# ndlongvn/MM-DTI

Measured on AMD Instinct MI355X. Metric: molecules/sec fwd+bwd (InfoNCE fine-tune), higher is better.
Workload: dtype fp16 forward / bf16 backward GEMM operands, fp32 accumulation

## Files before the change

### mm-dti_amd/csrc/gbf.hip

```cpp
#include "common.h"

namespace mmdti {

constexpr float GBF_A = 2.5066272160f;

__global__ __launch_bounds__(256) void gbf_fwd_kernel(const float* __restrict__ dist, const long long* __restrict__ et,
                                                      const float* __restrict__ mul, const float* __restrict__ bias,
                                                      const float* __restrict__ means, const float* __restrict__ stds,
                                                      long long P, int K, int E, bf16_t* __restrict__ feat) {
  const int kc = threadIdx.x & 15;
  const int pl = threadIdx.x >> 4;
  for (int k0 = kc * 8; k0 < K; k0 += 128) {
    float mu[8], sg[8], cf[8];
#pragma unroll
    for (int i = 0; i < 8; ++i) {
      mu[i] = means[k0 + i];
      sg[i] = fabsf(stds[k0 + i]) + 1e-5f;
      cf[i] = 1.0f / (GBF_A * sg[i]);
    }
    for (long long p = (long long)blockIdx.x * 16 + pl; p < P; p += (long long)gridDim.x * 16) {
      long long e = et[p];
      e = e < 0 ? 0 : (e >= E ? E - 1 : e);
      const float y = mul[e] * dist[p] + bias[e];
      uint32_t w[4];
#pragma unroll
      for (int i = 0; i < 4; ++i) {
        float z0 = (y - mu[2 * i]) / sg[2 * i], z1 = (y - mu[2 * i + 1]) / sg[2 * i + 1];
        float v0 = __expf(-0.5f * z0 * z0) * cf[2 * i], v1 = __expf(-0.5f * z1 * z1) * cf[2 * i + 1];
        w[i] = (uint32_t)f2bf(v0) | ((uint32_t)f2bf(v1) << 16);
      }
      *reinterpret_cast<uint4*>(feat + p * K + k0) = make_uint4(w[0], w[1], w[2], w[3]);
    }
  }
}

constexpr int GBF_MAXE = 4096;

__global__ __launch_bounds__(256) void gbf_bwd_kernel(const float* __restrict__ dist, const long long* __restrict__ et,
                                                      const float* __restrict__ mul, const float* __restrict__ bias,
                                                      const float* __restrict__ means, const float* __restrict__ stds,
                                                      long long P, int K, int E, const bf16_t* __restrict__ dfeat,
                                                      float* __restrict__ dmul, float* __restrict__ dbias,
                                                      float* __restrict__ dmeans, float* __restrict__ dstds) {
  extern __shared__ float hist[];
  const bool use_hist = E <= GBF_MAXE;
  if (use_hist) {
    for (int i = threadIdx.x; i < 2 * E; i += 256) hist[i] = 0.f;
    __syncthreads();
  }
  const int kc = threadIdx.x & 15, pl = threadIdx.x >> 4;
  for (int kb = 0; kb < K; kb += 128) {
    const int k0 = kb + kc * 8;
    const bool kact = k0 < K;
    float mu[8], sg[8], cf[8], amu[8], asg[8];
#pragma unroll
    for (int i = 0; i < 8; ++i) {
      mu[i] = kact ? means[k0 + i] : 0.f;
      sg[i] = kact ? fabsf(stds[k0 + i]) + 1e-5f : 1.f;
      cf[i] = 1.0f / (GBF_A * sg[i]);
      amu[i] = asg[i] = 0.f;
    }
    for (long long p0 = (long long)blockIdx.x * 16; p0 < P; p0 += (long long)gridDim.x * 16) {
      const long long p = p0 + pl;
      float dy = 0.f;
      long long e = 0;
      float d = 0.f;
      if (p < P && kact) {
        e = et[p];
        e = e < 0 ? 0 : (e >= E ? E - 1 : e);
        d = dist[p];
        const float y = mul[e] * d + bias[e];
        const uint4 u = *reinterpret_cast<const uint4*>(dfeat + p * K + k0);
        const uint32_t w[4] = {u.x, u.y, u.z, u.w};
#pragma unroll
        for (int i = 0; i < 8; ++i) {
          const float dv = __uint_as_float((i & 1) ? (w[i >> 1] & 0xffff0000u) : (w[i >> 1] << 16));
          const float z = (y - mu[i]) / sg[i];
          const float val = __expf(-0.5f * z * z) * cf[i];
          const float t = dv * val;
          const float zs = z / sg[i];
          dy -= t * zs;
          amu[i] += t * zs;
          asg[i] += t * (z * zs - 1.0f / sg[i]);
        }
      }
      dy += __shfl_xor(dy, 1, 64);
      dy += __shfl_xor(dy, 2, 64);
      dy += __shfl_xor(dy, 4, 64);
      dy += __shfl_xor(dy, 8, 64);
      if (kc == 0 && p < P) {
        if (use_hist) {
          atomicAdd(&hist[e], dy * d);
          atomicAdd(&hist[E + e], dy);
        } else {
          atomicAdd(dmul + e, dy * d);
          atomicAdd(dbias + e, dy);
        }
      }
    }
#pragma unroll
    for (int i = 0; i < 8; ++i) {
      float a = amu[i], s = asg[i];
      a += __shfl_xor(a, 16, 64); a += __shfl_xor(a, 32, 64);
      s += __shfl_xor(s, 16, 64); s += __shfl_xor(s, 32, 64);
      if ((threadIdx.x & 63) < 16 && kact) {
        atomicAdd(dmeans + k0 + i, a);
        atomicAdd(dstds + k0 + i, stds[k0 + i] < 0.f ? -s : s);
      }
    }
  }
  if (use_hist) {
    __syncthreads();
    for (int i = threadIdx.x; i < E; i += 256) {
      const float a = hist[i], b = hist[E + i];
      if (a != 0.f) atomicAdd(dmul + i, a);
      if (b != 0.f) atomicAdd(dbias + i, b);
    }
  }
}

__global__ __launch_bounds__(256) void pair_permute_fwd_kernel(const float* __restrict__ x, float* __restrict__ out,
                                                               int N, int H, int ld) {
  extern __shared__ float tile[];
  const int bi = blockIdx.x, b = bi / N, i = bi - b * N;
  const float* src = x + (long long)bi * N * H;
  const int HP = H + 1;
  for (int t = threadIdx.x; t < N * H; t += 256) tile[(t / H) * HP + (t % H)] = src[t];
  __syncthreads();
  for (int t = threadIdx.x; t < H * N; t += 256) {
    const int h = t / N, j = t - h * N;
    out[(((long long)b * H + h) * N + i) * ld + j] = tile[j * HP + h];
  }
}

__global__ __launch_bounds__(256) void pair_permute_bwd_kernel(const float* __restrict__ g, bf16_t* __restrict__ out,
                                                               int N, int H, int ld, int tiled) {
  extern __shared__ float tile[];
  const int bi = blockIdx.x, b = bi / N, i = bi - b * N;
  const int NP = N | 1;
  for (int t = threadIdx.x; t < H * N; t += 256) {
    const int h = t / N, j = t - h * N;
    const long long off = tiled ? (long long)(b * H + h) * pair_plane(N) + pair_off(N, i, j) : (((long long)b * H + h) * N + i) * ld + j;
    tile[h * NP + j] = g[off];
  }
  __syncthreads();
  bf16_t* dst = out + (long long)bi * N * H;
  for (int t = threadIdx.x; t < N * H; t += 256) {
    const int j = t / H, h = t - j * H;
    dst[t] = f2bf(tile[h * NP + j]);
  }
}

typedef __bf16 gbf16x8 __attribute__((ext_vector_type(8)));
typedef float gf32x4 __attribute__((ext_vector_type(4)));
constexpr int GBF_K = 128, GBF_F = 128, GBF_H = 64;
constexpr int GBF_WS = 136;

__device__ __forceinline__ gbf16x8 gbf_pack8(const float* v) {
  gbf16x8 r;
#pragma unroll
  for (int e = 0; e < 8; ++e) r[e] = (__bf16)v[e];
  return r;
}
__device__ __forceinline__ uint2 gbf_pack4(const gf32x4& a) {
  uint2 pk;
  pk.x = (uint32_t)f2bf(a[0]) | ((uint32_t)f2bf(a[1]) << 16);
  pk.y = (uint32_t)f2bf(a[2]) | ((uint32_t)f2bf(a[3]) << 16);
  return pk;
}

__device__ __forceinline__ int gbf_edge(const void* et, long long base, unsigned off, int esz) {
  const char* pb = reinterpret_cast<const char*>(et) + base * esz;
  const unsigned bo = off * (unsigned)esz;
  const int w = *reinterpret_cast<const int*>(pb + (bo & ~3u));
  return esz == 2 ? (int)(short)(w >> ((bo & 2u) * 8u)) : w;
}
__device__ __forceinline__ int gbf_edge(const void* et, long long p, int esz) { return gbf_edge(et, p, 0u, esz); }

typedef float gf32x2 __attribute__((ext_vector_type(2)));
constexpr float GBF_SQ = 0.84932180028801907f;

__device__ __forceinline__ gbf16x8 gbf_basis8(float y, const float* mu, const float* isq, const float* cf) {
  const gf32x4 m0 = *reinterpret_cast<const gf32x4*>(mu), m1 = *reinterpret_cast<const gf32x4*>(mu + 4);
  const gf32x4 s0 = *reinterpret_cast<const gf32x4*>(isq), s1 = *reinterpret_cast<const gf32x4*>(isq + 4);
  const gf32x4 c0 = *reinterpret_cast<const gf32x4*>(cf), c1 = *reinterpret_cast<const gf32x4*>(cf + 4);
  const gf32x2 yy = {y, y};
  float v[8];
#define GBF_B2(M, S, C, LO, OUT)                                                       \
  {                                                                                    \
    const gf32x2 z = (yy - gf32x2{M[LO], M[LO + 1]}) * gf32x2{S[LO], S[LO + 1]};       \
    const gf32x2 q = -(z * z);                                                         \
    const gf32x2 e = {__builtin_amdgcn_exp2f(q[0]), __builtin_amdgcn_exp2f(q[1])};     \
    const gf32x2 r = e * gf32x2{C[LO], C[LO + 1]};                                     \
    v[OUT] = r[0]; v[OUT + 1] = r[1];                                                  \
  }
  GBF_B2(m0, s0, c0, 0, 0) GBF_B2(m0, s0, c0, 2, 2) GBF_B2(m1, s1, c1, 0, 4) GBF_B2(m1, s1, c1, 2, 6)
#undef GBF_B2
  return gbf_pack8(v);
}

constexpr int GBF_FWD_MAXE = 4096;
__device__ __forceinline__ void gbf_put(float* p, float v) { *p = v; }
__device__ __forceinline__ void gbf_put(_Float16* p, float v) { *p = (_Float16)fminf(v, 65504.f); }
__device__ __forceinline__ float gbf_get(const float* p) { return *p; }
__device__ __forceinline__ float gbf_get(const __bf16* p) {
  return __builtin_bit_cast(float, (uint32_t)(*reinterpret_cast<const unsigned short*>(p)) << 16);
}

template <bool SAVE, bool TILED, typename OT>
__global__ __launch_bounds__(512, 2) void gbf_bias_fwd_kernel(const float* __restrict__ dist, const void* __restrict__ et, int esz,
                                                              const float* __restrict__ mul, const float* __restrict__ bias,
                                                              const float* __restrict__ means, const float* __restrict__ stds,
                                                              const bf16_t* __restrict__ W1, const float* __restrict__ b1,
                                                              const bf16_t* __restrict__ W2, const float* __restrict__ b2,
                                                              OT* __restrict__ out, bf16_t* __restrict__ feat_out,
                                                              bf16_t* __restrict__ u_out, bf16_t* __restrict__ h_out, int B, int N,
                                                              int ld, int E, int tpm, int ugrad, int ltab,
                                                              const int* __restrict__ tile_prefix, const int* __restrict__ row_blocks) {
  static_assert(TILED || sizeof(OT) == 4, "compact pair planes exist in the tiled layout only");
  extern __shared__ __attribute__((aligned(16))) unsigned char gbf_smem[];
  bf16_t* sW1 = reinterpret_cast<bf16_t*>(gbf_smem);
  bf16_t* sW2 = sW1 + GBF_F * GBF_WS;
  float* sMu = reinterpret_cast<float*>(sW2 + GBF_H * GBF_WS);
  float* sIq = sMu + GBF_K;
  float* sCf = sIq + GBF_K;
  float* sB1 = sCf + GBF_K;
  float* sB2 = sB1 + GBF_F;
  float* sMul = sB2 + GBF_H;
  float* sBia = sMul + E;
  const int tid = threadIdx.x, lane = tid & 63;
  for (int c = tid; c < GBF_F * (GBF_K / 8); c += 512) {
    const int row = c >> 4, col = (c & 15) * 8;
    *reinterpret_cast<uint4*>(sW1 + row * GBF_WS + col) = *reinterpret_cast<const uint4*>(W1 + row * GBF_K + col);
  }
  for (int c = tid; c < GBF_H * 32; c += 512) {
    const int row = c >> 5, pc = c & 31, u = pc >> 3, g = (pc >> 1) & 3, hf = pc & 1;
    *reinterpret_cast<uint2*>(sW2 + row * GBF_WS + 32 * u + 8 * g + 4 * hf) =
        *reinterpret_cast<const uint2*>(W2 + row * GBF_F + 32 * u + 16 * hf + 4 * g);
  }
  if (tid < GBF_K) {
    const float sg = fabsf(stds[tid]) + 1e-5f;
    sMu[tid] = means[tid];
    sIq[tid] = GBF_SQ / sg;
    sCf[tid] = 1.0f / (GBF_A * sg);
    sB1[tid] = b1[tid];
    if (tid < GBF_H) sB2[tid] = b2[tid];
  }
  if (ltab)
    for (int c = tid; c < E; c += 512) {
      sMul[c] = mul[c];
      sBia[c] = bias[c];
    }
  __syncthreads();
  const int g = lane >> 4, i = lane & 15;
  const bool rag = TILED && tile_prefix != nullptr;
  const int ntiles = rag ? tile_prefix[B] : B * tpm;
  const int nwaves = (int)gridDim.x * 8;
  int b_run = 0;
  const int nblk = (N + 3) >> 2;
  const long long plane = TILED ? pair_plane(N) : (long long)N * ld;
  auto fetch = [&](int tile, int& b, int& q, int& flags, unsigned& pl, int& e, float& d) {
    tile = __builtin_amdgcn_readfirstlane(tile < ntiles ? tile : ntiles - 1);
    int tq;
    if (rag) {
      while (b_run + 1 < B && tile >= tile_prefix[b_run + 1]) ++b_run;
      b = b_run;
      tq = tile - tile_prefix[b];
    } else {
      b = (int)((unsigned)tile / (unsigned)tpm);
      tq = tile - b * tpm;
    }
    int ii, jj;
    bool inplane = true, past = false;
    if (TILED) {
      const int rbk = (rag && row_blocks) ? row_blocks[b] : nblk;
      const int cb = (int)((unsigned)tq / (unsigned)rbk), rb = tq - cb * rbk;
      past = 4 * rb >= N || 4 * cb >= N;
      ii = 4 * rb + (i >> 2);
      jj = 4 * cb + (i & 3);
      inplane = ii < N;
      q = (int)pair_off(N, inplane ? ii : 0, jj);
    } else {
      q = tq * 16 + i;
      ii = (int)((unsigned)q / (unsigned)ld);
      jj = q - ii * ld;
      inplane = q < plane;
    }
    const bool valid = ii < N && jj < N;
    flags = (valid ? 1 : 0) | (inplane ? 2 : 0) | (past ? 4 : 0);
    pl = (unsigned)((valid ? ii : 0) * N + (valid ? jj : 0));
    const long long mol = (long long)b * N * N;
    const int e32 = gbf_edge(et, mol, pl, esz);
    e = e32 < 0 ? 0 : (e32 >= E ? E - 1 : e32);
    d = (dist + mol)[pl];
  };
  int b, q, flags, e, n_b, n_q, n_flags, n_e;
  unsigned pl, n_pl;
  float d, n_d;
  int tile = (int)blockIdx.x * 8 + (tid >> 6);
  fetch(tile, b, q, flags, pl, e, d);
  for (; tile < ntiles; tile += nwaves) {
    fetch(tile + nwaves, n_b, n_q, n_flags, n_pl, n_e, n_d);
    const bool valid = flags & 1, inplane = flags & 2, past = flags & 4;
    const float padv = TILED ? -INFINITY : 0.f;
    OT* ob = out + (long long)b * GBF_H * plane + q;
    if (TILED && past) {
    } else {
    const long long p = (long long)b * N * N + pl;
    const float y = ltab ? sMul[e] * d + sBia[e] : mul[e] * d + bias[e];
    gbf16x8 fB[4];
#pragma unroll
    for (int c = 0; c < 4; ++c) {
      const int k0 = 32 * c + 8 * g;
      fB[c] = gbf_basis8(y, sMu + k0, sIq + k0, sCf + k0);
      if (SAVE && valid) *reinterpret_cast<gbf16x8*>(feat_out + p * GBF_K + k0) = fB[c];
    }
    gbf16x8 hB[4];
#pragma unroll
    for (int u = 0; u < 4; ++u) {
      gf32x4 hv[2];
#pragma unroll
      for (int hf = 0; hf < 2; ++hf) {
        const int ft = 2 * u + hf;
        gf32x4 acc = {0.f, 0.f, 0.f, 0.f};
#pragma unroll
        for (int c = 0; c < 4; ++c) {
          const gbf16x8 wf = *reinterpret_cast<const gbf16x8*>(sW1 + (16 * ft + i) * GBF_WS + 32 * c + 8 * g);
          acc = __builtin_amdgcn_mfma_f32_16x16x32_bf16(wf, fB[c], acc, 0, 0, 0);
        }
        const gf32x4 bb = *reinterpret_cast<const gf32x4*>(sB1 + 16 * ft + 4 * g);
        acc += bb;
        if (SAVE && ugrad) {
          f32x2_t y0, g0, y1, g1;
          gelu_erf_both2(f32x2_t{acc[0], acc[1]}, y0, g0);
          gelu_erf_both2(f32x2_t{acc[2], acc[3]}, y1, g1);
          acc = gf32x4{y0[0], y0[1], y1[0], y1[1]};
          const gf32x4 gq = {g0[0], g0[1], g1[0], g1[1]};
          if (valid) *reinterpret_cast<uint2*>(u_out + p * GBF_F + 16 * ft + 4 * g) = gbf_pack4(gq);
        } else {
          if (SAVE && valid) *reinterpret_cast<uint2*>(u_out + p * GBF_F + 16 * ft + 4 * g) = gbf_pack4(acc);
          const f32x2_t y0 = gelu_erf2(f32x2_t{acc[0], acc[1]}), y1 = gelu_erf2(f32x2_t{acc[2], acc[3]});
          acc = gf32x4{y0[0], y0[1], y1[0], y1[1]};
        }
        if (SAVE && valid) *reinterpret_cast<uint2*>(h_out + p * GBF_F + 16 * ft + 4 * g) = gbf_pack4(acc);
        hv[hf] = acc;
        __builtin_amdgcn_sched_barrier(0);
      }
      float v[8] = {hv[0][0], hv[0][1], hv[0][2], hv[0][3], hv[1][0], hv[1][1], hv[1][2], hv[1][3]};
      hB[u] = gbf_pack8(v);
    }
#pragma unroll
    for (int ht = 0; ht < 4; ++ht) {
      gf32x4 acc = {0.f, 0.f, 0.f, 0.f};
#pragma unroll
      for (int u = 0; u < 4; ++u) {
        const gbf16x8 wf = *reinterpret_cast<const gbf16x8*>(sW2 + (16 * ht + i) * GBF_WS + 32 * u + 8 * g);
        acc = __builtin_amdgcn_mfma_f32_16x16x32_bf16(wf, hB[u], acc, 0, 0, 0);
      }
      const gf32x4 bb = *reinterpret_cast<const gf32x4*>(sB2 + 16 * ht + 4 * g);
      if (inplane) {
#pragma unroll
        for (int r = 0; r < 4; ++r) gbf_put(ob + (long long)(16 * ht + 4 * g + r) * plane, valid ? acc[r] + bb[r] : padv);
      }
      __builtin_amdgcn_sched_barrier(0);
    }
    }
    b = n_b; q = n_q; flags = n_flags; pl = n_pl; e = n_e; d = n_d;
  }
}

constexpr int GBF_W2S = 72;

template <bool TILED, typename GT>
__global__ __launch_bounds__(256, 2) void gbf_bias_bwd_kernel(const GT* __restrict__ gsrc, const float* __restrict__ dist,
                                                           const void* __restrict__ et, int esz, const float* __restrict__ mul,
                                                           const float* __restrict__ bias, const float* __restrict__ means,
                                                           const float* __restrict__ stds, const bf16_t* __restrict__ W1,
                                                           const bf16_t* __restrict__ W2, const bf16_t* __restrict__ u_in,
                                                           bf16_t* __restrict__ do_out, bf16_t* __restrict__ du_out,
                                                           float* __restrict__ dmul, float* __restrict__ dbias,
                                                           float* __restrict__ dmeans, float* __restrict__ dstds, int B, int N, int ld,
                                                           int E, int tpm, int ugrad) {
  extern __shared__ __attribute__((aligned(16))) unsigned char gbf_smem[];
  bf16_t* sW1T = reinterpret_cast<bf16_t*>(gbf_smem);
  bf16_t* sW2T = sW1T + GBF_K * GBF_WS;
  float* sMu = reinterpret_cast<float*>(sW2T + GBF_F * GBF_W2S);
  float* sIs = sMu + GBF_K;
  float* sCf = sIs + GBF_K;
  float* hist = sCf + GBF_K;
  float* sMul = hist + 2 * E;
  float* sBia = sMul + E;
  const int tid = threadIdx.x, lane = tid & 63;
  for (int c = tid; c < E; c += 256) {
    sMul[c] = mul[c];
    sBia[c] = bias[c];
  }
  for (int c = tid; c < GBF_K * GBF_F; c += 256) {
    const int f = c >> 7, k = c & 127;
    const int u = f >> 5, hf = (f >> 4) & 1, g = (f >> 2) & 3, e = f & 3;
    sW1T[k * GBF_WS + 32 * u + 8 * g + 4 * hf + e] = W1[c];
  }
  for (int c = tid; c < GBF_H * GBF_F; c += 256) {
    const int h = c >> 7, f = c & 127;
    sW2T[f * GBF_W2S + h] = W2[c];
  }
  if (tid < GBF_K) {
    const float sg = fabsf(stds[tid]) + 1e-5f;
    sMu[tid] = means[tid];
    sIs[tid] = 1.0f / sg;
    sCf[tid] = 1.0f / (GBF_A * sg);
  }
  for (int c = tid; c < 2 * E; c += 256) hist[c] = 0.f;
  __syncthreads();
  const int g = lane >> 4, i = lane & 15;
  const long long ntiles = (long long)B * tpm;
  const long long nwaves = (long long)gridDim.x * 4;
  const int nblk = (N + 3) >> 2;
  const long long plane = TILED ? pair_plane(N) : (long long)N * ld;
  gf32x4 amu[8], asg[8];
#pragma unroll
  for (int kt = 0; kt < 8; ++kt) amu[kt] = asg[kt] = gf32x4{0.f, 0.f, 0.f, 0.f};
  auto fetch = [&](long long tile, bool& act, bool& valid, long long& p, int& e, float& d, float (&gv)[16], uint2 (&up)[8]) {
    act = false;
    valid = false;
    p = 0;
    e = 0;
    d = 0.f;
    if (tile >= ntiles) return;
    const int b = (int)(tile / tpm);
    const int tq = (int)(tile - (long long)b * tpm);
    int q, ii, jj;
    if (TILED) {
      const int rb = tq / nblk, cb = tq - rb * nblk;
      if (4 * rb >= N || 4 * cb >= N) return;
      ii = 4 * rb + (i >> 2);
      jj = 4 * cb + (i & 3);
      q = (int)pair_off(N, ii < N ? ii : 0, jj);
    } else {
      q = tq * 16 + i;
      ii = q / ld;
      jj = q - ii * ld;
    }
    act = true;
    valid = ii < N && jj < N;
    p = ((long long)b * N + (valid ? ii : 0)) * N + (valid ? jj : 0);
    const int e32 = gbf_edge(et, p, esz);
    e = e32 < 0 ? 0 : (e32 >= E ? E - 1 : e32);
    d = dist[p];
    const GT* gp = gsrc + (long long)b * GBF_H * plane + (valid ? q : 0);
#pragma unroll
    for (int c = 0; c < 2; ++c)
#pragma unroll
      for (int j = 0; j < 8; ++j) gv[c * 8 + j] = valid ? gbf_get(gp + (long long)(32 * c + 8 * g + j) * plane) : 0.f;
#pragma unroll
    for (int ft = 0; ft < 8; ++ft) {
      up[ft] = make_uint2(0u, 0u);
      if (valid) up[ft] = *reinterpret_cast<const uint2*>(u_in + p * GBF_F + 16 * ft + 4 * g);
    }
  };
  bool act, valid, n_act, n_valid;
  long long p, n_p;
  int e, n_e;
  float d, n_d, gv[16], n_gv[16];
  uint2 upre[8], n_up[8];
  long long tile = (long long)blockIdx.x * 4 + (tid >> 6);
  fetch(tile, act, valid, p, e, d, gv, upre);
  for (; tile < ntiles; tile += nwaves) {
    fetch(tile + nwaves, n_act, n_valid, n_p, n_e, n_d, n_gv, n_up);
    if (act) {
    const float y = sMul[e] * d + sBia[e];
    gbf16x8 oB[2];
#pragma unroll
    for (int c = 0; c < 2; ++c) {
      oB[c] = gbf_pack8(gv + 8 * c);
      if (valid) *reinterpret_cast<gbf16x8*>(do_out + p * GBF_H + 32 * c + 8 * g) = oB[c];
    }
    gbf16x8 uB[4];
#pragma unroll
    for (int u = 0; u < 4; ++u) {
      gf32x4 dv[2];
#pragma unroll
      for (int hf = 0; hf < 2; ++hf) {
        const int ft = 2 * u + hf;
        gf32x4 acc = {0.f, 0.f, 0.f, 0.f};
#pragma unroll
        for (int c = 0; c < 2; ++c) {
          const gbf16x8 wf = *reinterpret_cast<const gbf16x8*>(sW2T + (16 * ft + i) * GBF_W2S + 32 * c + 8 * g);
          acc = __builtin_amdgcn_mfma_f32_16x16x32_bf16(wf, oB[c], acc, 0, 0, 0);
        }
        const uint2 up = upre[ft];
        if (ugrad) {
          acc[0] *= __uint_as_float(up.x << 16);
          acc[1] *= __uint_as_float(up.x & 0xffff0000u);
          acc[2] *= __uint_as_float(up.y << 16);
          acc[3] *= __uint_as_float(up.y & 0xffff0000u);
        } else {
          acc[0] *= gelu_erf_grad(__uint_as_float(up.x << 16));
          acc[1] *= gelu_erf_grad(__uint_as_float(up.x & 0xffff0000u));
          acc[2] *= gelu_erf_grad(__uint_as_float(up.y << 16));
          acc[3] *= gelu_erf_grad(__uint_as_float(up.y & 0xffff0000u));
        }
        if (valid) *reinterpret_cast<uint2*>(du_out + p * GBF_F + 16 * ft + 4 * g) = gbf_pack4(acc);
        dv[hf] = acc;
        __builtin_amdgcn_sched_barrier(0);
      }
      float v[8] = {dv[0][0], dv[0][1], dv[0][2], dv[0][3], dv[1][0], dv[1][1], dv[1][2], dv[1][3]};
      uB[u] = gbf_pack8(v);
    }
    float dy = 0.f;
#pragma unroll
    for (int kt = 0; kt < 8; ++kt) {
      gf32x4 acc = {0.f, 0.f, 0.f, 0.f};
#pragma unroll
      for (int u = 0; u < 4; ++u) {
        const gbf16x8 wf = *reinterpret_cast<const gbf16x8*>(sW1T + (16 * kt + i) * GBF_WS + 32 * u + 8 * g);
        acc = __builtin_amdgcn_mfma_f32_16x16x32_bf16(wf, uB[u], acc, 0, 0, 0);
      }
      const gf32x4 mu = *reinterpret_cast<const gf32x4*>(sMu + 16 * kt + 4 * g);
      const gf32x4 is = *reinterpret_cast<const gf32x4*>(sIs + 16 * kt + 4 * g);
      const gf32x4 cf = *reinterpret_cast<const gf32x4*>(sCf + 16 * kt + 4 * g);
#pragma unroll
      for (int r = 0; r < 4; ++r) {
        const float dvr = __uint_as_float(((uint32_t)f2bf(acc[r])) << 16);
        const float z = (y - mu[r]) * is[r];
        const float val = __expf(-0.5f * z * z) * cf[r];
        const float t = valid ? dvr * val : 0.f;
        const float zs = z * is[r];
        dy -= t * zs;
        amu[kt][r] += t * zs;
        asg[kt][r] += t * (z * zs - is[r]);
      }
      __builtin_amdgcn_sched_barrier(0);
    }
    dy += __shfl_xor(dy, 16, 64);
    dy += __shfl_xor(dy, 32, 64);
    if (g == 0 && valid) {
      atomicAdd(&hist[e], dy * d);
      atomicAdd(&hist[E + e], dy);
    }
    }
    act = n_act; valid = n_valid; p = n_p; e = n_e; d = n_d;
#pragma unroll
    for (int j = 0; j < 16; ++j) gv[j] = n_gv[j];
#pragma unroll
    for (int j = 0; j < 8; ++j) upre[j] = n_up[j];
  }
#pragma unroll
  for (int kt = 0; kt < 8; ++kt)
#pragma unroll
    for (int r = 0; r < 4; ++r) {
      float a = amu[kt][r], sgv = asg[kt][r];
      a += __shfl_xor(a, 1, 64); a += __shfl_xor(a, 2, 64); a += __shfl_xor(a, 4, 64); a += __shfl_xor(a, 8, 64);
      sgv += __shfl_xor(sgv, 1, 64); sgv += __shfl_xor(sgv, 2, 64); sgv += __shfl_xor(sgv, 4, 64); sgv += __shfl_xor(sgv, 8, 64);
      if (i == 0) {
        const int k = 16 * kt + 4 * g + r;
        atomicAdd(dmeans + k, a);
        atomicAdd(dstds + k, stds[k] < 0.f ? -sgv : sgv);
      }
    }
  __syncthreads();
  for (int c = tid; c < E; c += 256) {
    const float a = hist[c], bb = hist[E + c];
    if (a != 0.f) atomicAdd(dmul + c, a);
    if (bb != 0.f) atomicAdd(dbias + c, bb);
  }
}

constexpr int GBF_LW = 144;
constexpr int GBF_FULL_MAXE = 1536;
constexpr int GBF_SLAB_B1 = GBF_F * GBF_K + GBF_H * GBF_F, GBF_SLAB_B2 = GBF_SLAB_B1 + GBF_F, GBF_SLAB_MU = GBF_SLAB_B2 + GBF_H,
              GBF_SLAB_SG = GBF_SLAB_MU + GBF_K, GBF_SLAB = GBF_SLAB_SG + GBF_K;
constexpr size_t gbf_full_smem(int E) {
  return (size_t)(GBF_F * GBF_LW + GBF_F * GBF_W2S + 2 * 128 * GBF_LW) * 2 + (size_t)(4 * GBF_K + GBF_F + 2 * 128 + 4 * E) * 4;
}

typedef short gs16x4 __attribute__((ext_vector_type(4)));
typedef short gs16x8 __attribute__((ext_vector_type(8)));
typedef __attribute__((address_space(3))) gs16x4 glds_s16x4;
__device__ __forceinline__ gbf16x8 gbf_tr8(const bf16_t* a0, const bf16_t* a1) {
  const gs16x4 lo = __builtin_amdgcn_ds_read_tr16_b64_v4i16((glds_s16x4*)a0);
  const gs16x4 hi = __builtin_amdgcn_ds_read_tr16_b64_v4i16((glds_s16x4*)a1);
  const gs16x8 v = __builtin_shufflevector(lo, hi, 0, 1, 2, 3, 4, 5, 6, 7);
  return __builtin_bit_cast(gbf16x8, v);
}

template <bool TILED, typename GT>
__global__ __launch_bounds__(512, 1) void gbf_bias_bwd_full_kernel(
    const GT* __restrict__ gsrc, const float* __restrict__ dist, const void* __restrict__ et, int esz, const float* __restrict__ mul,
    const float* __restrict__ bias, const float* __restrict__ means, const float* __restrict__ stds, const bf16_t* __restrict__ W1,
    const float* __restrict__ b1, const bf16_t* __restrict__ W2, float* __restrict__ dW1, float* __restrict__ db1, float* __restrict__ dW2,
    float* __restrict__ db2, float* __restrict__ dmul, float* __restrict__ dbias, float* __restrict__ dmeans, float* __restrict__ dstds, int B,
    int N, int ld, int E, int tpm, const int* __restrict__ tile_prefix, const int* __restrict__ row_blocks, float* __restrict__ slab) {
  extern __shared__ __attribute__((aligned(16))) unsigned char gbf_smem[];
  bf16_t* sW1 = reinterpret_cast<bf16_t*>(gbf_smem);
  bf16_t* sW2T = sW1 + GBF_F * GBF_LW;
  bf16_t* T0 = sW2T + GBF_F * GBF_W2S;
  bf16_t* T1 = T0 + 128 * GBF_LW;
  float* sMu = reinterpret_cast<float*>(T1 + 128 * GBF_LW);
  float* sIs = sMu + GBF_K;
  float* sCf = sIs + GBF_K;
  float* sIq = sCf + GBF_K;
  float* sB1 = sIq + GBF_K;
  float* sY = sB1 + GBF_F;
  float* sDy = sY + 128;
  float* hist = sDy + 128;
  float* sMul = hist + 2 * E;
  float* sBia = sMul + E;
  const int tid = threadIdx.x, lane = tid & 63, wave = tid >> 6;
  for (int c = tid; c < E; c += 512) {
    sMul[c] = mul[c];
    sBia[c] = bias[c];
  }
  for (int c = tid; c < GBF_F * (GBF_K / 8); c += 512) {
    const int row = c >> 4, col = (c & 15) * 8;
    *reinterpret_cast<uint4*>(sW1 + row * GBF_LW + col) = *reinterpret_cast<const uint4*>(W1 + row * GBF_K + col);
  }
  for (int c = tid; c < GBF_H * GBF_F; c += 512) {
    const int h = c >> 7, f = c & 127;
    sW2T[f * GBF_W2S + h] = W2[c];
  }
  if (tid < GBF_K) {
    const float sg = fabsf(stds[tid]) + 1e-5f;
    sMu[tid] = means[tid];
    sIs[tid] = 1.0f / sg;
    sCf[tid] = 1.0f / (GBF_A * sg);
    sIq[tid] = GBF_SQ / sg;
    sB1[tid] = b1[tid];
    sDy[tid] = 0.f;
  }
  for (int c = tid; c < 2 * E; c += 512) hist[c] = 0.f;
  __syncthreads();
  const int g = lane >> 4, i = lane & 15;
  const int ploc = 16 * wave + i;
  const int pswz = ((ploc >> 3) & 1) << 6;
#define GBF_SWZ(lo, hi, c) ((c) < 64 ? (lo) + (c) : (hi) + ((c) - 64))
  bf16_t* const r0lo = T0 + ploc * GBF_LW + pswz;
  bf16_t* const r0hi = T0 + ploc * GBF_LW + (64 ^ pswz);
  bf16_t* const r1lo = r0lo + 128 * GBF_LW;
  bf16_t* const r1hi = r0hi + 128 * GBF_LW;
  const int tswz = (g & 1) << 6;
  const int trow = (8 * g + (i >> 2)) * GBF_LW + 4 * (i & 3);
  const bf16_t* const t0lo = T0 + trow + tswz;
  const bf16_t* const t0hi = T0 + trow + (64 ^ tswz);
  const bf16_t* const t1lo = t0lo + 128 * GBF_LW;
  const bf16_t* const t1hi = t0hi + 128 * GBF_LW;
  const bf16_t* const t0w = T0 + trow + ((16 * wave) ^ tswz);
  const bf16_t* const t1w = t0w + 128 * GBF_LW;
  const int rswz = ((i >> 3) & 1) << 6;
  const bf16_t* const d1lo = T1 + i * GBF_LW + 8 * g + rswz;
  const bf16_t* const d1hi = T1 + i * GBF_LW + 8 * g + (64 ^ rswz);
  unsigned o_w1row = (unsigned)(i * GBF_LW + 8 * g) * 2;
  unsigned o_w2row = (unsigned)(GBF_F * GBF_LW + i * GBF_W2S + 8 * g) * 2;
  unsigned o_w1tr = (unsigned)((8 * g + (i >> 2)) * GBF_LW + 16 * wave + 4 * (i & 3)) * 2;
  const unsigned o_f32 = (unsigned)(GBF_F * GBF_LW + GBF_F * GBF_W2S + 2 * 128 * GBF_LW) * 2;
  unsigned o_gconst = o_f32 + (unsigned)(8 * g) * 4;
  unsigned o_b1row = o_f32 + (unsigned)(4 * GBF_K + 4 * g) * 4;
  unsigned o_kconst = o_f32 + (unsigned)(16 * wave + 4 * g) * 4;
  const bool rag = TILED && tile_prefix != nullptr;
  const int ntiles = rag ? tile_prefix[B] : B * tpm;
  int b_run = 0;
  const int nb = (N + 3) >> 2;
  const long long plane = TILED ? pair_plane(N) : (long long)N * ld;
  gf32x4 amu = {0.f, 0.f, 0.f, 0.f}, asg = {0.f, 0.f, 0.f, 0.f};
  gf32x4 aW1[8], aW2[4], aB1 = {0.f, 0.f, 0.f, 0.f}, aB2 = {0.f, 0.f, 0.f, 0.f};
#pragma unroll
  for (int t = 0; t < 8; ++t) aW1[t] = gf32x4{0.f, 0.f, 0.f, 0.f};
#pragma unroll
  for (int t = 0; t < 4; ++t) aW2[t] = gf32x4{0.f, 0.f, 0.f, 0.f};
  const gs16x8 o16 = {0x3F80, 0x3F80, 0x3F80, 0x3F80, 0x3F80, 0x3F80, 0x3F80, 0x3F80};
  const gbf16x8 ones = __builtin_bit_cast(gbf16x8, o16);

  auto fetch = [&](int tile, bool& act, bool& valid, float& d, int& e, float (&gv)[16]) {
    tile = __builtin_amdgcn_readfirstlane(tile);
    act = tile < ntiles;
    tile = act ? tile : ntiles - 1;
    int b, tq;
    if (rag) {
      while (b_run + 1 < B && tile >= tile_prefix[b_run + 1]) ++b_run;
      b = b_run;
      tq = tile - tile_prefix[b];
    } else {
      b = (int)((unsigned)tile / (unsigned)tpm);
      tq = tile - b * tpm;
    }
    int q, ii, jj;
    if (TILED) {
      const int rbk = (rag && row_blocks) ? row_blocks[b] : nb;
      const int cb = (int)((unsigned)tq / (unsigned)rbk), rb = tq - cb * rbk;
      ii = 4 * rb + (i >> 2);
      jj = 4 * cb + (i & 3);
      q = (int)pair_off(N, ii < N ? ii : 0, jj);
    } else {
      q = tq * 16 + i;
      ii = (int)((unsigned)q / (unsigned)ld);
      jj = q - ii * ld;
    }
    valid = act && ii < N && jj < N;
    const long long mol = (long long)b * N * N;
    const unsigned pl = (unsigned)((valid ? ii : 0) * N + (valid ? jj : 0));
    const int e32 = gbf_edge(et, mol, pl, esz);
    e = e32 < 0 ? 0 : (e32 >= E ? E - 1 : e32);
    d = (dist + mol)[pl];
    const GT* mb = gsrc + (long long)b * GBF_H * plane;
    const unsigned voff = (unsigned)(8 * g) * (unsigned)plane + (unsigned)(valid ? q : 0);
#pragma unroll
    for (int c = 0; c < 2; ++c)
#pragma unroll
      for (int j = 0; j < 8; ++j) gv[c * 8 + j] = gbf_get(mb + (long long)(32 * c + j) * plane + voff);
  };

  bool act, valid, n_act, n_valid;
  float d, n_d, gv[16], n_gv[16];
  int e, n_e;
  const int stride = (int)gridDim.x * 8;
  int tile = (int)blockIdx.x * 8 + wave;
  fetch(tile, act, valid, d, e, gv);
  for (int base = (int)blockIdx.x * 8; base < ntiles; base += stride, tile += stride) {
    asm volatile("" : "+v"(o_w1row), "+v"(o_w2row), "+v"(o_w1tr), "+v"(o_gconst), "+v"(o_b1row), "+v"(o_kconst));
    const bf16_t* w1row = reinterpret_cast<const bf16_t*>(gbf_smem + o_w1row);
    const bf16_t* w2row = reinterpret_cast<const bf16_t*>(gbf_smem + o_w2row);
    const bf16_t* w1tr = reinterpret_cast<const bf16_t*>(gbf_smem + o_w1tr);
    const float* gconst = reinterpret_cast<const float*>(gbf_smem + o_gconst);
    const float* b1row = reinterpret_cast<const float*>(gbf_smem + o_b1row);
    const float* kconst = reinterpret_cast<const float*>(gbf_smem + o_kconst);
    fetch(tile + stride, n_act, n_valid, n_d, n_e, n_gv);
    constexpr bool SPLIT_G = sizeof(GT) == 4;
    gbf16x8 oB[2], oL[2], hB[4];
    if (!valid) {
#pragma unroll
      for (int j = 0; j < 16; ++j) gv[j] = 0.f;
    }
    oB[0] = gbf_pack8(gv);
    oB[1] = gbf_pack8(gv + 8);
    if constexpr (SPLIT_G) {
      float lo[16];
#pragma unroll
      for (int j = 0; j < 16; ++j) lo[j] = gv[j] - (float)oB[j >> 3][j & 7];
      oL[0] = gbf_pack8(lo);
      oL[1] = gbf_pack8(lo + 8);
    }
    const float y = sMul[e] * d + sBia[e];
    if (g == 0) sY[ploc] = y;
    if (act) {
      gbf16x8 fB[4];
#pragma unroll
      for (int c = 0; c < 4; ++c) {
        const float* gc = gconst + 32 * c;
        fB[c] = gbf_basis8(y, gc, gc + 3 * GBF_K, gc + 2 * GBF_K);
        *reinterpret_cast<gbf16x8*>(GBF_SWZ(r0lo, r0hi, 32 * c) + 8 * g) = fB[c];
      }
#pragma unroll
      for (int u = 0; u < 4; ++u) {
        gf32x4 hv[2];
#pragma unroll
        for (int hf = 0; hf < 2; ++hf) {
          const int ft = 2 * u + hf;
          gf32x4 acc = {0.f, 0.f, 0.f, 0.f}, ua = {0.f, 0.f, 0.f, 0.f};
#pragma unroll
          for (int c = 0; c < 2; ++c) {
            const gbf16x8 wf = *reinterpret_cast<const gbf16x8*>(w2row + 16 * ft * GBF_W2S + 32 * c);
            acc = __builtin_amdgcn_mfma_f32_16x16x32_bf16(wf, oB[c], acc, 0, 0, 0);
            if constexpr (SPLIT_G) acc = __builtin_amdgcn_mfma_f32_16x16x32_bf16(wf, oL[c], acc, 0, 0, 0);
          }
#pragma unroll
          for (int c = 0; c < 4; ++c) {
            const gbf16x8 wf = *reinterpret_cast<const gbf16x8*>(w1row + 16 * ft * GBF_LW + 32 * c);
            ua = __builtin_amdgcn_mfma_f32_16x16x32_bf16(wf, fB[c], ua, 0, 0, 0);
          }
          ua += *reinterpret_cast<const gf32x4*>(b1row + 16 * ft);
          {
            f32x2_t y0, g0, y1, g1;
            gelu_erf_both2(f32x2_t{ua[0], ua[1]}, y0, g0);
            gelu_erf_both2(f32x2_t{ua[2], ua[3]}, y1, g1);
            hv[hf] = gf32x4{y0[0], y0[1], y1[0], y1[1]};
            const uint2 gb = gbf_pack4(gf32x4{g0[0], g0[1], g1[0], g1[1]});
            acc[0] *= __uint_as_float(gb.x << 16);
            acc[1] *= __uint_as_float(gb.x & 0xffff0000u);
            acc[2] *= __uint_as_float(gb.y << 16);
            acc[3] *= __uint_as_float(gb.y & 0xffff0000u);
          }
          *reinterpret_cast<uint2*>(GBF_SWZ(r1lo, r1hi, 16 * ft) + 4 * g) = gbf_pack4(acc);
          __builtin_amdgcn_sched_barrier(0);
        }
        float w[8] = {hv[0][0], hv[0][1], hv[0][2], hv[0][3], hv[1][0], hv[1][1], hv[1][2], hv[1][3]};
        hB[u] = gbf_pack8(w);
      }
    } else {
      const uint4 z4 = make_uint4(0u, 0u, 0u, 0u);
#pragma unroll
      for (int c = 0; c < 4; ++c) {
        *reinterpret_cast<uint4*>(GBF_SWZ(r0lo, r0hi, 32 * c) + 8 * g) = z4;
        *reinterpret_cast<uint4*>(GBF_SWZ(r1lo, r1hi, 32 * c) + 8 * g) = z4;
        hB[c] = __builtin_bit_cast(gbf16x8, z4);
      }
    }
    __syncthreads();
#define GBF_TFRAG(P, S) gbf_tr8((P) + 32 * (S) * GBF_LW, (P) + (32 * (S) + 4) * GBF_LW)
#pragma unroll
    for (int sstep = 0; sstep < 4; ++sstep) {
      const gbf16x8 fa = GBF_TFRAG(t1w, sstep);
      aB1 = __builtin_amdgcn_mfma_f32_16x16x32_bf16(fa, ones, aB1, 0, 0, 0);
#pragma unroll
      for (int kb = 0; kb < 8; ++kb) {
        const gbf16x8 fb = GBF_TFRAG(GBF_SWZ(t0lo, t0hi, 16 * kb), sstep);
        aW1[kb] = __builtin_amdgcn_mfma_f32_16x16x32_bf16(fa, fb, aW1[kb], 0, 0, 0);
      }
    }
    {
      gbf16x8 wfr[4];
#pragma unroll
      for (int u = 0; u < 4; ++u) {
        wfr[u] = gbf_tr8(w1tr + 32 * u * GBF_LW, w1tr + (32 * u + 4) * GBF_LW);
      }
      const gf32x4 kmu = *reinterpret_cast<const gf32x4*>(kconst);
      const gf32x4 kis = *reinterpret_cast<const gf32x4*>(kconst + GBF_K);
      const gf32x4 kcf = *reinterpret_cast<const gf32x4*>(kconst + 2 * GBF_K);
#pragma unroll 1
      for (int j = 0; j < 8; ++j) {
        gf32x4 acc = {0.f, 0.f, 0.f, 0.f};
#pragma unroll
        for (int u = 0; u < 4; ++u) {
          const gbf16x8 dub = *reinterpret_cast<const gbf16x8*>(GBF_SWZ(d1lo, d1hi, 32 * u) + 16 * j * GBF_LW);
          acc = __builtin_amdgcn_mfma_f32_16x16x32_bf16(wfr[u], dub, acc, 0, 0, 0);
        }
        const float yj = sY[16 * j + i];
        const gf32x2 yy = {yj, yj};
        gf32x2 dy2 = {0.f, 0.f};
#define GBF_G2(LO, DV0, DV1)                                                                                   \
        {                                                                                                      \
          const gf32x2 is2 = {kis[LO], kis[LO + 1]};                                                           \
          const gf32x2 z = (yy - gf32x2{kmu[LO], kmu[LO + 1]}) * is2;                                          \
          const gf32x2 qq = (z * z) * (-0.72134752044448170f);                               \
          const gf32x2 val = gf32x2{__builtin_amdgcn_exp2f(qq[0]), __builtin_amdgcn_exp2f(qq[1])} * gf32x2{kcf[LO], kcf[LO + 1]}; \
          const gf32x2 t = gf32x2{DV0, DV1} * val;          \
          const gf32x2 zs = z * is2;                                                                           \
          const gf32x2 tz = t * zs;                                                                            \
          dy2 -= tz;                                                                                           \
          amu[LO] += tz[0]; amu[LO + 1] += tz[1];                                                              \
          const gf32x2 w = t * (z * zs - is2);                                                                 \
          asg[LO] += w[0]; asg[LO + 1] += w[1];                                                                \
        }
        GBF_G2(0, acc[0], acc[1])
        GBF_G2(2, acc[2], acc[3])
#undef GBF_G2
        float dy = dy2[0] + dy2[1];
        dy += __shfl_xor(dy, 16, 64);
        dy += __shfl_xor(dy, 32, 64);
        if (g == 0) atomicAdd(&sDy[16 * j + i], dy);
      }
    }
    __syncthreads();
#pragma unroll
    for (int u = 0; u < 4; ++u) {
      const uint4 hw = __builtin_bit_cast(uint4, hB[u]);
      *reinterpret_cast<uint2*>(GBF_SWZ(r0lo, r0hi, 32 * u) + 4 * g) = make_uint2(hw.x, hw.y);
      *reinterpret_cast<uint2*>(GBF_SWZ(r0lo, r0hi, 32 * u + 16) + 4 * g) = make_uint2(hw.z, hw.w);
    }
    *reinterpret_cast<gbf16x8*>(r1lo + 8 * g) = oB[0];
    *reinterpret_cast<gbf16x8*>(r1lo + 32 + 8 * g) = oB[1];
    if constexpr (SPLIT_G) {
      *reinterpret_cast<gbf16x8*>(r1hi + 8 * g) = oL[0];
      *reinterpret_cast<gbf16x8*>(r1hi + 32 + 8 * g) = oL[1];
    }
    if (g == 0) {
      const float dyv = sDy[ploc];
      sDy[ploc] = 0.f;
      if (valid) {
        atomicAdd(&hist[e], dyv * d);
        atomicAdd(&hist[E + e], dyv);
      }
    }
    __syncthreads();
#pragma unroll
    for (int sstep = 0; sstep < 4; ++sstep) {
      const gbf16x8 fb = GBF_TFRAG(t0w, sstep);
#pragma unroll
      for (int hb = 0; hb < 4; ++hb) {
        const gbf16x8 fa = GBF_TFRAG(t1lo + 16 * hb, sstep);
        aW2[hb] = __builtin_amdgcn_mfma_f32_16x16x32_bf16(fa, fb, aW2[hb], 0, 0, 0);
        if constexpr (SPLIT_G) {
          const gbf16x8 fl = GBF_TFRAG(t1hi + 16 * hb, sstep);
          aW2[hb] = __builtin_amdgcn_mfma_f32_16x16x32_bf16(fl, fb, aW2[hb], 0, 0, 0);
        }
      }
      const gbf16x8 fo = GBF_TFRAG(t1lo + 16 * (wave & 3), sstep);
      aB2 = __builtin_amdgcn_mfma_f32_16x16x32_bf16(fo, ones, aB2, 0, 0, 0);
      if constexpr (SPLIT_G) {
        const gbf16x8 fol = GBF_TFRAG(t1hi + 16 * (wave & 3), sstep);
        aB2 = __builtin_amdgcn_mfma_f32_16x16x32_bf16(fol, ones, aB2, 0, 0, 0);
      }
    }
#undef GBF_TFRAG
#undef GBF_SWZ
    __syncthreads();
    act = n_act; valid = n_valid; d = n_d; e = n_e;
#pragma unroll
    for (int j = 0; j < 16; ++j) gv[j] = n_gv[j];
  }
  float* const sl = slab ? slab + (long long)blockIdx.x * (GBF_SLAB + 2 * E) : nullptr;
#pragma unroll
  for (int kb = 0; kb < 8; ++kb)
#pragma unroll
    for (int r = 0; r < 4; ++r) {
      const int o = (16 * wave + 4 * g + r) * GBF_K + 16 * kb + i;
      if (sl) sl[o] = aW1[kb][r]; else atomicAdd(dW1 + o, aW1[kb][r]);
    }
#pragma unroll
  for (int hb = 0; hb < 4; ++hb)
#pragma unroll
    for (int r = 0; r < 4; ++r) {
      const int o = (16 * hb + 4 * g + r) * GBF_F + 16 * wave + i;
      if (sl) sl[GBF_F * GBF_K + o] = aW2[hb][r]; else atomicAdd(dW2 + o, aW2[hb][r]);
    }
  if (i == 0) {
#pragma unroll
    for (int r = 0; r < 4; ++r) {
      const int o = 16 * wave + 4 * g + r;
      if (sl) {
        sl[GBF_SLAB_B1 + o] = aB1[r];
        if (wave < 4) sl[GBF_SLAB_B2 + o] = aB2[r];
      } else {
        atomicAdd(db1 + o, aB1[r]);
        if (wave < 4) atomicAdd(db2 + o, aB2[r]);
      }
    }
  }
#pragma unroll
  for (int r = 0; r < 4; ++r) {
    float a = amu[r], sgv = asg[r];
    a += __shfl_xor(a, 1, 64); a += __shfl_xor(a, 2, 64); a += __shfl_xor(a, 4, 64); a += __shfl_xor(a, 8, 64);
    sgv += __shfl_xor(sgv, 1, 64); sgv += __shfl_xor(sgv, 2, 64); sgv += __shfl_xor(sgv, 4, 64); sgv += __shfl_xor(sgv, 8, 64);
    if (i == 0) {
      const int k = 16 * wave + 4 * g + r;
      const float ds = stds[k] < 0.f ? -sgv : sgv;
      if (sl) { sl[GBF_SLAB_MU + k] = a; sl[GBF_SLAB_SG + k] = ds; }
      else { atomicAdd(dmeans + k, a); atomicAdd(dstds + k, ds); }
    }
  }
  __syncthreads();
  for (int c = tid; c < E; c += 512) {
    const float a = hist[c], bb = hist[E + c];
    if (sl) { sl[GBF_SLAB + c] = a; sl[GBF_SLAB + E + c] = bb; }
    else {
      if (a != 0.f) atomicAdd(dmul + c, a);
      if (bb != 0.f) atomicAdd(dbias + c, bb);
    }
  }
}

__global__ __launch_bounds__(256) void gbf_slab_reduce_kernel(const float* __restrict__ slab, int nwg, int E, float* __restrict__ dW1, float* __restrict__ db1,
                                                              float* __restrict__ dW2, float* __restrict__ db2, float* __restrict__ dmul,
                                                              float* __restrict__ dbias, float* __restrict__ dmeans, float* __restrict__ dstds) {
  __shared__ float part[4][64];
  const int SL = GBF_SLAB + 2 * E;
  const int el = threadIdx.x & 63, q = threadIdx.x >> 6;
  const int e = blockIdx.x * 64 + el;
  const int per = (nwg + 3) / 4, w0 = q * per, w1 = min(nwg, w0 + per);
  float t = 0.f;
  if (e < SL) {
    const float* sp = slab + (long long)w0 * SL + e;
    int w = w0;
    for (; w + 8 <= w1; w += 8, sp += 8ll * SL) {
      float v[8];
#pragma unroll
      for (int j = 0; j < 8; ++j) v[j] = sp[(long long)j * SL];
#pragma unroll
      for (int j = 0; j < 8; ++j) t += v[j];
    }
    for (; w < w1; ++w, sp += SL) t += *sp;
  }
  part[q][el] = t;
  __syncthreads();
  if (q != 0 || e >= SL) return;
  t = ((part[0][el] + part[1][el]) + part[2][el]) + part[3][el];
  float* dst;
  if (e < GBF_F * GBF_K) dst = dW1 + e;
  else if (e < GBF_SLAB_B1) dst = dW2 + (e - GBF_F * GBF_K);
  else if (e < GBF_SLAB_B2) dst = db1 + (e - GBF_SLAB_B1);
  else if (e < GBF_SLAB_MU) dst = db2 + (e - GBF_SLAB_B2);
  else if (e < GBF_SLAB_SG) dst = dmeans + (e - GBF_SLAB_MU);
  else if (e < GBF_SLAB) dst = dstds + (e - GBF_SLAB_SG);
  else if (e < GBF_SLAB + E) dst = dmul + (e - GBF_SLAB);
  else dst = dbias + (e - GBF_SLAB - E);
  *dst += t;
}

__global__ __launch_bounds__(256) void pair_untile_bwd_kernel(const float* __restrict__ g, bf16_t* __restrict__ out, int N, int H,
                                                              int nt) {
  extern __shared__ bf16_t ptile[];
  const int HP = H + 2;
  const int t = blockIdx.x % nt, qb = (blockIdx.x / nt) % nt, b = blockIdx.x / (nt * nt);
  const long long plane = pair_plane(N);
  const int vr = min(16, N - qb * 16);
  const float* src = g + (long long)b * H * plane + (long long)qb * 16 * pair_n4(N) + vr * 16 * t;
  for (int e = threadIdx.x; e < H * 64; e += 256) {
    const int h = e >> 6, l = e & 63;
    const int q = l & 15, k0 = (l >> 4) * 4;
    float4 v = make_float4(0.f, 0.f, 0.f, 0.f);
    if (q < vr && t * 16 + k0 < N) v = *reinterpret_cast<const float4*>(src + (long long)h * plane + ((l >> 4) * vr + q) * 4);
    bf16_t* d = ptile + (q * 16 + k0) * HP + h;
    d[0] = f2bf(v.x); d[HP] = f2bf(v.y); d[2 * HP] = f2bf(v.z); d[3 * HP] = f2bf(v.w);
  }
  __syncthreads();
  for (int e = threadIdx.x; e < 256 * (H / 2); e += 256) {
    const int pr = e / (H / 2), h2 = e - pr * (H / 2);
    const int i = qb * 16 + (pr >> 4), j = t * 16 + (pr & 15);
    if (i < N && j < N)
      *reinterpret_cast<uint32_t*>(out + (((long long)b * N + i) * N + j) * H + 2 * h2) =
          *reinterpret_cast<const uint32_t*>(ptile + pr * HP + 2 * h2);
  }
}

}
using namespace mmdti;

static int gbf_check(const char* fn, long long P, int K, int E) {
  MMDTI_REQUIRE(P > 0 && K > 0 && K % 8 == 0 && E > 0, "%s: need P>0, K%%8==0, E>0 (K=%d)", fn, K);
  return MMDTI_OK;
}

extern "C" int mmdti_gbf_features_fwd(mmdti_stream_t stream, const float* dist, const long long* edge_type,
                                      const float* mul, const float* bias, const float* means, const float* stds,
                                      long long P, int K, int E, void* feat_bf16) {
  if (int e = gbf_check("gbf_features_fwd", P, K, E)) return e;
  MMDTI_REQUIRE(dist && edge_type && mul && bias && means && stds && feat_bf16, "gbf_features_fwd: null pointer");
  MMDTI_REQUIRE(aligned16(feat_bf16), "gbf_features_fwd: feat must be 16-byte aligned");
  long long blocks = (P + 15) / 16;
  if (blocks > 256 * 32) blocks = 256 * 32;
  hipLaunchKernelGGL(gbf_fwd_kernel, dim3((unsigned)blocks), dim3(256), 0, (hipStream_t)stream, dist, edge_type, mul,
                     bias, means, stds, P, K, E, (bf16_t*)feat_bf16);
  MMDTI_LAUNCH_CHECK();
  return MMDTI_OK;
}

extern "C" int mmdti_gbf_features_bwd(mmdti_stream_t stream, const float* dist, const long long* edge_type,
                                      const float* mul, const float* bias, const float* means, const float* stds,
                                      long long P, int K, int E, const void* dfeat_bf16, float* dmul, float* dbias,
                                      float* dmeans, float* dstds) {
  if (int e = gbf_check("gbf_features_bwd", P, K, E)) return e;
  MMDTI_REQUIRE(dist && edge_type && mul && bias && means && stds && dfeat_bf16 && dmul && dbias && dmeans && dstds,
                "gbf_features_bwd: null pointer");
  MMDTI_REQUIRE(aligned16(dfeat_bf16), "gbf_features_bwd: dfeat must be 16-byte aligned");
  long long blocks = (P + 15) / 16;
  if (blocks > 256 * 8) blocks = 256 * 8;
  const size_t smem = E <= GBF_MAXE ? 2 * (size_t)E * sizeof(float) : 0;
  hipLaunchKernelGGL(gbf_bwd_kernel, dim3((unsigned)blocks), dim3(256), smem, (hipStream_t)stream, dist, edge_type,
                     mul, bias, means, stds, P, K, E, (const bf16_t*)dfeat_bf16, dmul, dbias, dmeans, dstds);
  MMDTI_LAUNCH_CHECK();
  return MMDTI_OK;
}

extern "C" int mmdti_pair_permute_fwd(mmdti_stream_t stream, const float* x, float* out, int B, int N, int H, int ld) {
  MMDTI_REQUIRE(x && out && B > 0 && N > 0 && H > 0 && ld >= N, "pair_permute_fwd: bad arguments");
  const size_t smem = (size_t)N * (H + 1) * sizeof(float);
  MMDTI_REQUIRE(smem <= 64 * 1024, "pair_permute_fwd: N*H too large for the LDS tile (N=%d,H=%d)", N, H);
  hipLaunchKernelGGL(pair_permute_fwd_kernel, dim3(B * N), dim3(256), smem, (hipStream_t)stream, x, out, N, H, ld);
  MMDTI_LAUNCH_CHECK();
  return MMDTI_OK;
}

extern "C" int mmdti_pair_permute_bwd(mmdti_stream_t stream, const float* g, void* out_bf16, int B, int N, int H,
                                      int ld, int tiled) {
  MMDTI_REQUIRE(g && out_bf16 && B > 0 && N > 0 && H > 0 && ld >= N, "pair_permute_bwd: bad arguments");
  if (tiled && H % 2 == 0 && (size_t)256 * (H + 2) * 2 <= 64 * 1024 && aligned16(g)) {
    const int nt = (N + 15) / 16;
    hipLaunchKernelGGL(pair_untile_bwd_kernel, dim3(B * nt * nt), dim3(256), (size_t)256 * (H + 2) * 2, (hipStream_t)stream, g,
                       (bf16_t*)out_bf16, N, H, nt);
    MMDTI_LAUNCH_CHECK();
    return MMDTI_OK;
  }
  const size_t smem = (size_t)H * (N | 1) * sizeof(float);
  MMDTI_REQUIRE(smem <= 64 * 1024, "pair_permute_bwd: N*H too large for the LDS tile (N=%d,H=%d)", N, H);
  hipLaunchKernelGGL(pair_permute_bwd_kernel, dim3(B * N), dim3(256), smem, (hipStream_t)stream, g, (bf16_t*)out_bf16,
                     N, H, ld, tiled);
  MMDTI_LAUNCH_CHECK();
  return MMDTI_OK;
}

static int edge_bytes_ok(int eb) { return eb == 8 || eb == 4 || eb == 2; }

extern "C" int mmdti_gbf_bias_fwd(mmdti_stream_t stream, const float* dist, const void* edge_type, int edge_bytes, const float* mul,
                                  const float* bias, const float* means, const float* stds, const void* w1_bf16,
                                  const float* b1, const void* w2_bf16, const float* b2, int B, int N, int ld, int K, int F,
                                  int H, int E, void* out, void* feat_bf16, void* u_bf16, void* h_bf16, int flags,
                                  const int* tile_prefix, const int* row_blocks) {
  const int tiled = flags & 1, ugrad = (flags >> 1) & 1, compact = (flags >> 2) & 1;
  MMDTI_REQUIRE(!compact || tiled, "gbf_bias_fwd: compact planes (flags bit 2) exist in the tiled layout only");
  MMDTI_REQUIRE(!tile_prefix || tiled, "gbf_bias_fwd: tile_prefix (ragged batches) needs the tiled pair layout");
  MMDTI_REQUIRE(!row_blocks || tile_prefix, "gbf_bias_fwd: row_blocks (packed token rows) comes with tile_prefix");
  MMDTI_REQUIRE(dist && edge_type && mul && bias && means && stds && w1_bf16 && b1 && w2_bf16 && b2 && out, "gbf_bias_fwd: null argument");
  MMDTI_REQUIRE(edge_bytes_ok(edge_bytes), "gbf_bias_fwd: edge types must be int64, int32 or int16 (edge_bytes=%d)", edge_bytes);
  MMDTI_REQUIRE(K == GBF_K && F == GBF_F && H == GBF_H, "gbf_bias_fwd: built for %d gaussians, %d hidden, %d heads (got %d,%d,%d)",
                GBF_K, GBF_F, GBF_H, K, F, H);
  MMDTI_REQUIRE(B > 0 && N > 0 && ld >= N && ld % 4 == 0 && E > 0, "gbf_bias_fwd: bad shape");
  MMDTI_REQUIRE(aligned16(w1_bf16) && aligned16(w2_bf16) && aligned16(out), "gbf_bias_fwd: 16-byte alignment required");
  const bool save = feat_bf16 || u_bf16 || h_bf16;
  MMDTI_REQUIRE(!save || (feat_bf16 && u_bf16 && h_bf16 && aligned16(feat_bf16) && aligned16(u_bf16) && aligned16(h_bf16)),
                "gbf_bias_fwd: the three saved intermediates come together, 16-byte aligned");
  const int nb4 = (N + 3) / 4;
  const int tpm = tiled ? nb4 * nb4 : cdiv((long long)N * ld, 16);
  const long long ntiles = (long long)B * tpm;
  MMDTI_REQUIRE(ntiles < (1ll << 30) && (long long)N * N < (1ll << 30), "gbf_bias_fwd: batch too large for 32-bit tile indices");
  const int grid = (int)((ntiles + 7) / 8 < 512 ? (ntiles + 7) / 8 : 512);
  const int ltab = E <= GBF_FWD_MAXE ? 1 : 0;
  const size_t smem = (size_t)(GBF_F + GBF_H) * GBF_WS * 2 + (size_t)(3 * GBF_K + GBF_F + GBF_H + (ltab ? 2 * E : 0)) * 4;
  static bool attr_done = false;
  if (!attr_done) {
    const int cap = (int)((size_t)(GBF_F + GBF_H) * GBF_WS * 2 + (size_t)(3 * GBF_K + GBF_F + GBF_H + 2 * GBF_FWD_MAXE) * 4);
    const void* fns[6] = {reinterpret_cast<const void*>(gbf_bias_fwd_kernel<true, true, float>), reinterpret_cast<const void*>(gbf_bias_fwd_kernel<true, false, float>),
                          reinterpret_cast<const void*>(gbf_bias_fwd_kernel<false, true, float>), reinterpret_cast<const void*>(gbf_bias_fwd_kernel<false, false, float>),
                          reinterpret_cast<const void*>(gbf_bias_fwd_kernel<true, true, _Float16>), reinterpret_cast<const void*>(gbf_bias_fwd_kernel<false, true, _Float16>)};
    for (int f = 0; f < 6; ++f)
      if (hipFuncSetAttribute(fns[f], hipFuncAttributeMaxDynamicSharedMemorySize, cap) != hipSuccess) {
        set_error("gbf_bias_fwd: hipFuncSetAttribute failed");
        return MMDTI_ERR_LAUNCH;
      }
    attr_done = true;
  }
#define GBF_L(SAVE, TILED, OT)                                                                                                      \
  hipLaunchKernelGGL((gbf_bias_fwd_kernel<SAVE, TILED, OT>), dim3(grid), dim3(512), smem, (hipStream_t)stream, dist, edge_type, edge_bytes, mul, bias, \
                     means, stds, (const bf16_t*)w1_bf16, b1, (const bf16_t*)w2_bf16, b2, (OT*)out, (bf16_t*)feat_bf16, (bf16_t*)u_bf16, \
                     (bf16_t*)h_bf16, B, N, ld, E, tpm, ugrad, ltab, tile_prefix, row_blocks)
  if (compact) { if (save) GBF_L(true, true, _Float16); else GBF_L(false, true, _Float16); }
  else if (save) { if (tiled) GBF_L(true, true, float); else GBF_L(true, false, float); }
  else           { if (tiled) GBF_L(false, true, float); else GBF_L(false, false, float); }
#undef GBF_L
  MMDTI_LAUNCH_CHECK();
  return MMDTI_OK;
}

extern "C" int mmdti_gbf_bias_bwd(mmdti_stream_t stream, const void* g, const float* dist, const void* edge_type, int edge_bytes,
                                  const float* mul, const float* bias, const float* means, const float* stds,
                                  const void* w1_bf16, const void* w2_bf16, const void* u_bf16, int B, int N, int ld, int K,
                                  int F, int H, int E, int flags, void* do_bf16, void* du_bf16, float* dmul, float* dbias,
                                  float* dmeans, float* dstds) {
  const int tiled = flags & 1, ugrad = (flags >> 1) & 1, compact = (flags >> 2) & 1;
  MMDTI_REQUIRE(!compact || tiled, "gbf_bias_bwd: compact planes (flags bit 2) exist in the tiled layout only");
  MMDTI_REQUIRE(g && dist && edge_type && mul && bias && means && stds && w1_bf16 && w2_bf16 && u_bf16 && do_bf16 && du_bf16 && dmul &&
                    dbias && dmeans && dstds, "gbf_bias_bwd: null argument");
  MMDTI_REQUIRE(K == GBF_K && F == GBF_F && H == GBF_H, "gbf_bias_bwd: built for %d gaussians, %d hidden, %d heads (got %d,%d,%d)",
                GBF_K, GBF_F, GBF_H, K, F, H);
  MMDTI_REQUIRE(B > 0 && N > 0 && ld >= N && ld % 4 == 0 && E > 0 && E <= GBF_MAXE, "gbf_bias_bwd: bad shape (E <= %d)", GBF_MAXE);
  MMDTI_REQUIRE(edge_bytes_ok(edge_bytes), "gbf_bias_bwd: edge types must be int64, int32 or int16 (edge_bytes=%d)", edge_bytes);
  MMDTI_REQUIRE(aligned16(u_bf16) && aligned16(do_bf16) && aligned16(du_bf16), "gbf_bias_bwd: 16-byte alignment required");
  const int nb4 = (N + 3) / 4;
  const int tpm = tiled ? nb4 * nb4 : cdiv((long long)N * ld, 16);
  const long long ntiles = (long long)B * tpm;
  const int grid = (int)(ntiles / 4 + 1 < 1024 ? ntiles / 4 + 1 : 1024);
  const size_t smem = (size_t)GBF_K * GBF_WS * 2 + (size_t)GBF_F * GBF_W2S * 2 + (size_t)(3 * GBF_K + 4 * E) * 4;
  MMDTI_REQUIRE(smem <= 96 * 1024, "gbf_bias_bwd: %d edge types do not fit the LDS tables", E);
  static bool attr_done = false;
  if (!attr_done) {
    if (hipFuncSetAttribute(reinterpret_cast<const void*>(gbf_bias_bwd_kernel<true, float>), hipFuncAttributeMaxDynamicSharedMemorySize, 96 * 1024) != hipSuccess ||
        hipFuncSetAttribute(reinterpret_cast<const void*>(gbf_bias_bwd_kernel<false, float>), hipFuncAttributeMaxDynamicSharedMemorySize, 96 * 1024) != hipSuccess ||
        hipFuncSetAttribute(reinterpret_cast<const void*>(gbf_bias_bwd_kernel<true, __bf16>), hipFuncAttributeMaxDynamicSharedMemorySize, 96 * 1024) != hipSuccess) {
      set_error("gbf_bias_bwd: hipFuncSetAttribute failed");
      return MMDTI_ERR_LAUNCH;
    }
    attr_done = true;
  }
#define GBF_B(TILED, GT)                                                                                                      \
  hipLaunchKernelGGL((gbf_bias_bwd_kernel<TILED, GT>), dim3(grid), dim3(256), smem, (hipStream_t)stream, (const GT*)g, dist, edge_type, edge_bytes, mul, bias, \
                     means, stds, (const bf16_t*)w1_bf16, (const bf16_t*)w2_bf16, (const bf16_t*)u_bf16, (bf16_t*)do_bf16,    \
                     (bf16_t*)du_bf16, dmul, dbias, dmeans, dstds, B, N, ld, E, tpm, ugrad)
  if (compact) GBF_B(true, __bf16); else if (tiled) GBF_B(true, float); else GBF_B(false, float);
#undef GBF_B
  MMDTI_LAUNCH_CHECK();
  return MMDTI_OK;
}

extern "C" int mmdti_gbf_bias_bwd_full(mmdti_stream_t stream, const void* g, const float* dist, const void* edge_type, int edge_bytes,
                                       const float* mul, const float* bias, const float* means, const float* stds, const void* w1_bf16,
                                       const float* b1, const void* w2_bf16, int B, int N, int ld, int K, int F, int H, int E, int flags,
                                       float* dw1, float* db1, float* dw2, float* db2, float* dmul, float* dbias, float* dmeans,
                                       float* dstds, const int* tile_prefix, const int* row_blocks, void* workspace, long long workspace_bytes) {
  const int tiled = flags & 1, compact = (flags >> 2) & 1;
  MMDTI_REQUIRE(!compact || tiled, "gbf_bias_bwd_full: compact planes (flags bit 2) exist in the tiled layout only");
  MMDTI_REQUIRE(!tile_prefix || tiled, "gbf_bias_bwd_full: tile_prefix (ragged batches) needs the tiled pair layout");
  MMDTI_REQUIRE(!row_blocks || tile_prefix, "gbf_bias_bwd_full: row_blocks (packed token rows) comes with tile_prefix");
  MMDTI_REQUIRE(g && dist && edge_type && mul && bias && means && stds && w1_bf16 && b1 && w2_bf16 && dw1 && db1 && dw2 && db2 && dmul && dbias &&
                    dmeans && dstds, "gbf_bias_bwd_full: null argument");
  MMDTI_REQUIRE(edge_bytes_ok(edge_bytes), "gbf_bias_bwd_full: edge types must be int64, int32 or int16 (edge_bytes=%d)", edge_bytes);
  MMDTI_REQUIRE(K == GBF_K && F == GBF_F && H == GBF_H, "gbf_bias_bwd_full: built for %d gaussians, %d hidden, %d heads (got %d,%d,%d)",
                GBF_K, GBF_F, GBF_H, K, F, H);
  MMDTI_REQUIRE(B > 0 && N > 0 && ld >= N && ld % 4 == 0 && E > 0 && E <= GBF_FULL_MAXE, "gbf_bias_bwd_full: bad shape (E <= %d)", GBF_FULL_MAXE);
  MMDTI_REQUIRE((long long)N * ld * GBF_H < (1ll << 29) && (long long)B * N * ld / 16 < (1ll << 30), "gbf_bias_bwd_full: batch too large for 32-bit tile offsets");
  MMDTI_REQUIRE(aligned16(w1_bf16), "gbf_bias_bwd_full: W1 must be 16-byte aligned");
  const int nb = (N + 3) / 4;
  const int tpm = tiled ? nb * nb : cdiv((long long)N * ld, 16);
  const long long ntiles = (long long)B * tpm;
  const int grid = (int)((ntiles + 7) / 8 < 256 ? (ntiles + 7) / 8 : 256);
  const size_t smem = gbf_full_smem(E);
  static bool attr_done = false;
  if (!attr_done) {
    const int cap = (int)gbf_full_smem(GBF_FULL_MAXE);
    if (hipFuncSetAttribute(reinterpret_cast<const void*>(gbf_bias_bwd_full_kernel<true, float>), hipFuncAttributeMaxDynamicSharedMemorySize, cap) != hipSuccess ||
        hipFuncSetAttribute(reinterpret_cast<const void*>(gbf_bias_bwd_full_kernel<false, float>), hipFuncAttributeMaxDynamicSharedMemorySize, cap) != hipSuccess ||
        hipFuncSetAttribute(reinterpret_cast<const void*>(gbf_bias_bwd_full_kernel<true, __bf16>), hipFuncAttributeMaxDynamicSharedMemorySize, cap) != hipSuccess) {
      set_error("gbf_bias_bwd_full: hipFuncSetAttribute failed");
      return MMDTI_ERR_LAUNCH;
    }
    attr_done = true;
  }
#define GBF_FB(TILED, GT)                                                                                                          \
  hipLaunchKernelGGL((gbf_bias_bwd_full_kernel<TILED, GT>), dim3(grid), dim3(512), smem, (hipStream_t)stream, (const GT*)g, dist, edge_type, edge_bytes, mul, \
                     bias, means, stds, (const bf16_t*)w1_bf16, b1, (const bf16_t*)w2_bf16, dw1, db1, dw2, db2, dmul, dbias, dmeans, dstds, B, \
                     N, ld, E, tpm, tile_prefix, row_blocks, slab)
  const long long SL = GBF_SLAB + 2 * (long long)E;
  float* slab = (workspace && aligned16(workspace) && workspace_bytes >= (long long)grid * SL * 4) ? reinterpret_cast<float*>(workspace) : nullptr;
  if (compact) GBF_FB(true, __bf16); else if (tiled) GBF_FB(true, float); else GBF_FB(false, float);
#undef GBF_FB
  if (slab)
    hipLaunchKernelGGL(gbf_slab_reduce_kernel, dim3(cdiv(SL, 64)), dim3(256), 0, (hipStream_t)stream, slab, grid, E, dw1, db1, dw2, db2, dmul, dbias, dmeans, dstds);
  MMDTI_LAUNCH_CHECK();
  return MMDTI_OK;
}

extern "C" int mmdti_gbf_bias_bwd_full_workspace(int E) { return (int)(256ll * (GBF_SLAB + 2ll * (E > 0 ? E : 0)) * 4); }
```

Baseline: 5038.

## Warp-specialize GBF bias backward into producer and MFMA consumer waves

The fused GBF bias backward kernel now splits its eight waves into roles. Four producer waves fetch gradients, compute the basis, the hidden activations and the GELU-scaled upstream gradient for 64 pairs, then stage them in shared memory. Four consumer waves run the weight-gradient MFMAs, with each wave owning a 32-wide slice of F. Producers prefetch and compute the next tile while consumers work on the current one, and the edge histogram fold is deferred through a double-buffered parity slot. The aim is to overlap the elementwise and global-load work with the matrix accumulation. The cost is more barriers, a smaller tile per block, a larger grid, and doubled accumulator registers in the consumer waves.

Measured after the change: 5089, median of 6. +1.0%, better.

```diff
diff --git a/mm-dti_amd/csrc/gbf.hip b/mm-dti_amd/csrc/gbf.hip
--- a/mm-dti_amd/csrc/gbf.hip
+++ b/mm-dti_amd/csrc/gbf.hip
@@ -567,11 +567,12 @@
 }
 
 constexpr int GBF_LW = 144;
+constexpr int GBF_BP = 64;
 constexpr int GBF_FULL_MAXE = 1536;
 constexpr int GBF_SLAB_B1 = GBF_F * GBF_K + GBF_H * GBF_F, GBF_SLAB_B2 = GBF_SLAB_B1 + GBF_F, GBF_SLAB_MU = GBF_SLAB_B2 + GBF_H,
               GBF_SLAB_SG = GBF_SLAB_MU + GBF_K, GBF_SLAB = GBF_SLAB_SG + GBF_K;
 constexpr size_t gbf_full_smem(int E) {
-  return (size_t)(GBF_F * GBF_LW + GBF_F * GBF_W2S + 2 * 128 * GBF_LW) * 2 + (size_t)(4 * GBF_K + GBF_F + 2 * 128 + 4 * E) * 4;
+  return (size_t)(GBF_F * GBF_LW + GBF_F * GBF_W2S + 4 * GBF_BP * GBF_LW) * 2 + (size_t)(4 * GBF_K + GBF_F + 9 * GBF_BP + 4 * E) * 4;
 }
 
 typedef short gs16x4 __attribute__((ext_vector_type(4)));
@@ -592,21 +593,23 @@
     float* __restrict__ db2, float* __restrict__ dmul, float* __restrict__ dbias, float* __restrict__ dmeans, float* __restrict__ dstds, int B,
     int N, int ld, int E, int tpm, const int* __restrict__ tile_prefix, const int* __restrict__ row_blocks, float* __restrict__ slab) {
   extern __shared__ __attribute__((aligned(16))) unsigned char gbf_smem[];
+  constexpr int TS = GBF_BP * GBF_LW;
   bf16_t* sW1 = reinterpret_cast<bf16_t*>(gbf_smem);
   bf16_t* sW2T = sW1 + GBF_F * GBF_LW;
   bf16_t* T0 = sW2T + GBF_F * GBF_W2S;
-  bf16_t* T1 = T0 + 128 * GBF_LW;
-  float* sMu = reinterpret_cast<float*>(T1 + 128 * GBF_LW);
+  float* sMu = reinterpret_cast<float*>(T0 + 4 * TS);
   float* sIs = sMu + GBF_K;
   float* sCf = sIs + GBF_K;
   float* sIq = sCf + GBF_K;
   float* sB1 = sIq + GBF_K;
   float* sY = sB1 + GBF_F;
-  float* sDy = sY + 128;
-  float* hist = sDy + 128;
+  float* sDy = sY + GBF_BP;
+  float* sEd = sDy + 4 * GBF_BP;
+  float* hist = sEd + 4 * GBF_BP;
   float* sMul = hist + 2 * E;
   float* sBia = sMul + E;
-  const int tid = threadIdx.x, lane = tid & 63, wave = tid >> 6;
+  const int tid = threadIdx.x, lane = tid & 63;
+  const int wave = __builtin_amdgcn_readfirstlane(tid >> 6);
   for (int c = tid; c < E; c += 512) {
     sMul[c] = mul[c];
     sBia[c] = bias[c];
@@ -626,318 +629,371 @@
     sCf[tid] = 1.0f / (GBF_A * sg);
     sIq[tid] = GBF_SQ / sg;
     sB1[tid] = b1[tid];
-    sDy[tid] = 0.f;
   }
   for (int c = tid; c < 2 * E; c += 512) hist[c] = 0.f;
   __syncthreads();
   const int g = lane >> 4, i = lane & 15;
-  const int ploc = 16 * wave + i;
-  const int pswz = ((ploc >> 3) & 1) << 6;
-#define GBF_SWZ(lo, hi, c) ((c) < 64 ? (lo) + (c) : (hi) + ((c) - 64))
-  bf16_t* const r0lo = T0 + ploc * GBF_LW + pswz;
-  bf16_t* const r0hi = T0 + ploc * GBF_LW + (64 ^ pswz);
-  bf16_t* const r1lo = r0lo + 128 * GBF_LW;
-  bf16_t* const r1hi = r0hi + 128 * GBF_LW;
-  const int tswz = (g & 1) << 6;
-  const int trow = (8 * g + (i >> 2)) * GBF_LW + 4 * (i & 3);
-  const bf16_t* const t0lo = T0 + trow + tswz;
-  const bf16_t* const t0hi = T0 + trow + (64 ^ tswz);
-  const bf16_t* const t1lo = t0lo + 128 * GBF_LW;
-  const bf16_t* const t1hi = t0hi + 128 * GBF_LW;
-  const bf16_t* const t0w = T0 + trow + ((16 * wave) ^ tswz);
-  const bf16_t* const t1w = t0w + 128 * GBF_LW;
-  const int rswz = ((i >> 3) & 1) << 6;
-  const bf16_t* const d1lo = T1 + i * GBF_LW + 8 * g + rswz;
-  const bf16_t* const d1hi = T1 + i * GBF_LW + 8 * g + (64 ^ rswz);
-  unsigned o_w1row = (unsigned)(i * GBF_LW + 8 * g) * 2;
-  unsigned o_w2row = (unsigned)(GBF_F * GBF_LW + i * GBF_W2S + 8 * g) * 2;
-  unsigned o_w1tr = (unsigned)((8 * g + (i >> 2)) * GBF_LW + 16 * wave + 4 * (i & 3)) * 2;
-  const unsigned o_f32 = (unsigned)(GBF_F * GBF_LW + GBF_F * GBF_W2S + 2 * 128 * GBF_LW) * 2;
-  unsigned o_gconst = o_f32 + (unsigned)(8 * g) * 4;
-  unsigned o_b1row = o_f32 + (unsigned)(4 * GBF_K + 4 * g) * 4;
-  unsigned o_kconst = o_f32 + (unsigned)(16 * wave + 4 * g) * 4;
+  const int q4 = wave & 3;
+  const unsigned o_f32 = (unsigned)(GBF_F * GBF_LW + GBF_F * GBF_W2S + 4 * TS) * 2;
   const bool rag = TILED && tile_prefix != nullptr;
   const int ntiles = rag ? tile_prefix[B] : B * tpm;
-  int b_run = 0;
-  const int nb = (N + 3) >> 2;
-  const long long plane = TILED ? pair_plane(N) : (long long)N * ld;
-  gf32x4 amu = {0.f, 0.f, 0.f, 0.f}, asg = {0.f, 0.f, 0.f, 0.f};
-  gf32x4 aW1[8], aW2[4], aB1 = {0.f, 0.f, 0.f, 0.f}, aB2 = {0.f, 0.f, 0.f, 0.f};
-#pragma unroll
-  for (int t = 0; t < 8; ++t) aW1[t] = gf32x4{0.f, 0.f, 0.f, 0.f};
-#pragma unroll
-  for (int t = 0; t < 4; ++t) aW2[t] = gf32x4{0.f, 0.f, 0.f, 0.f};
+  const int stride = (int)gridDim.x * 4;
   const gs16x8 o16 = {0x3F80, 0x3F80, 0x3F80, 0x3F80, 0x3F80, 0x3F80, 0x3F80, 0x3F80};
   const gbf16x8 ones = __builtin_bit_cast(gbf16x8, o16);
-
-  auto fetch = [&](int tile, bool& act, bool& valid, float& d, int& e, float (&gv)[16]) {
-    tile = __builtin_amdgcn_readfirstlane(tile);
-    act = tile < ntiles;
-    tile = act ? tile : ntiles - 1;
-    int b, tq;
-    if (rag) {
-      while (b_run + 1 < B && tile >= tile_prefix[b_run + 1]) ++b_run;
-      b = b_run;
-      tq = tile - tile_prefix[b];
-    } else {
-      b = (int)((unsigned)tile / (unsigned)tpm);
-      tq = tile - b * tpm;
-    }
-    int q, ii, jj;
-    if (TILED) {
-      const int rbk = (rag && row_blocks) ? row_blocks[b] : nb;
-      const int cb = (int)((unsigned)tq / (unsigned)rbk), rb = tq - cb * rbk;
-      ii = 4 * rb + (i >> 2);
-      jj = 4 * cb + (i & 3);
-      q = (int)pair_off(N, ii < N ? ii : 0, jj);
-    } else {
-      q = tq * 16 + i;
-      ii = (int)((unsigned)q / (unsigned)ld);
-      jj = q - ii * ld;
-    }
-    valid = act && ii < N && jj < N;
-    const long long mol = (long long)b * N * N;
-    const unsigned pl = (unsigned)((valid ? ii : 0) * N + (valid ? jj : 0));
-    const int e32 = gbf_edge(et, mol, pl, esz);
-    e = e32 < 0 ? 0 : (e32 >= E ? E - 1 : e32);
-    d = (dist + mol)[pl];
-    const GT* mb = gsrc + (long long)b * GBF_H * plane;
-    const unsigned voff = (unsigned)(8 * g) * (unsigned)plane + (unsigned)(valid ? q : 0);
-#pragma unroll
-    for (int c = 0; c < 2; ++c)
-#pragma unroll
-      for (int j = 0; j < 8; ++j) gv[c * 8 + j] = gbf_get(mb + (long long)(32 * c + j) * plane + voff);
-  };
-
-  bool act, valid, n_act, n_valid;
-  float d, n_d, gv[16], n_gv[16];
-  int e, n_e;
-  const int stride = (int)gridDim.x * 8;
-  int tile = (int)blockIdx.x * 8 + wave;
-  fetch(tile, act, valid, d, e, gv);
-  for (int base = (int)blockIdx.x * 8; base < ntiles; base += stride, tile += stride) {
-    asm volatile("" : "+v"(o_w1row), "+v"(o_w2row), "+v"(o_w1tr), "+v"(o_gconst), "+v"(o_b1row), "+v"(o_kconst));
-    const bf16_t* w1row = reinterpret_cast<const bf16_t*>(gbf_smem + o_w1row);
-    const bf16_t* w2row = reinterpret_cast<const bf16_t*>(gbf_smem + o_w2row);
-    const bf16_t* w1tr = reinterpret_cast<const bf16_t*>(gbf_smem + o_w1tr);
-    const float* gconst = reinterpret_cast<const float*>(gbf_smem + o_gconst);
-    const float* b1row = reinterpret_cast<const float*>(gbf_smem + o_b1row);
-    const float* kconst = reinterpret_cast<const float*>(gbf_smem + o_kconst);
+#define GBF_SWZ(lo, hi, c) ((c) < 64 ? (lo) + (c) : (hi) + ((c) - 64))
+  if (wave < 4) {
+    int b_run = 0;
+    const int nb = (N + 3) >> 2;
+    const long long plane = TILED ? pair_plane(N) : (long long)N * ld;
+    const int ploc = 16 * q4 + i;
+    const int pswz = ((ploc >> 3) & 1) << 6;
+    bf16_t* const r0lo = T0 + ploc * GBF_LW + pswz;
+    bf16_t* const r0hi = T0 + ploc * GBF_LW + (64 ^ pswz);
+    bf16_t* const r1lo = r0lo + TS;
+    bf16_t* const r1hi = r0hi + TS;
+    bf16_t* const r2lo = r0lo + 2 * TS;
+    bf16_t* const r2hi = r0hi + 2 * TS;
+    bf16_t* const r3lo = r0lo + 3 * TS;
+    bf16_t* const r3hi = r0hi + 3 * TS;
+    unsigned o_w1row = (unsigned)(i * GBF_LW + 8 * g) * 2;
+    unsigned o_w2row = (unsigned)(GBF_F * GBF_LW + i * GBF_W2S + 8 * g) * 2;
+    unsigned o_gconst = o_f32 + (unsigned)(8 * g) * 4;
+    unsigned o_b1row = o_f32 + (unsigned)(4 * GBF_K + 4 * g) * 4;
+
+    auto fetch = [&](int tile, bool& act, bool& valid, float& d, int& e, float (&gv)[16]) {
+      tile = __builtin_amdgcn_readfirstlane(tile);
+      act = tile < ntiles;
+      tile = act ? tile : ntiles - 1;
+      int b, tq;
+      if (rag) {
+        while (b_run + 1 < B && tile >= tile_prefix[b_run + 1]) ++b_run;
+        b = b_run;
+        tq = tile - tile_prefix[b];
+      } else {
+        b = (int)((unsigned)tile / (unsigned)tpm);
+        tq = tile - b * tpm;
+      }
+      int q, ii, jj;
+      if (TILED) {
+        const int rbk = (rag && row_blocks) ? row_blocks[b] : nb;
+        const int cb = (int)((unsigned)tq / (unsigned)rbk), rb = tq - cb * rbk;
+        ii = 4 * rb + (i >> 2);
+        jj = 4 * cb + (i & 3);
+        q = (int)pair_off(N, ii < N ? ii : 0, jj);
+      } else {
+        q = tq * 16 + i;
+        ii = (int)((unsigned)q / (unsigned)ld);
+        jj = q - ii * ld;
+      }
+      valid = act && ii < N && jj < N;
+      const long long mol = (long long)b * N * N;
+      const unsigned pl = (unsigned)((valid ? ii : 0) * N + (valid ? jj : 0));
+      const int e32 = gbf_edge(et, mol, pl, esz);
+      e = e32 < 0 ? 0 : (e32 >= E ? E - 1 : e32);
+      d = (dist + mol)[pl];
+      const GT* mb = gsrc + (long long)b * GBF_H * plane;
+      const unsigned voff = (unsigned)(8 * g) * (unsigned)plane + (unsigned)(valid ? q : 0);
+#pragma unroll
+      for (int c = 0; c < 2; ++c)
+#pragma unroll
+        for (int j = 0; j < 8; ++j) gv[c * 8 + j] = gbf_get(mb + (long long)(32 * c + j) * plane + voff);
+    };
+
+    constexpr bool SPLIT_G = sizeof(GT) == 4;
+    bool act, valid, n_act, n_valid;
+    float d, n_d, gv[16], n_gv[16];
+    int e, n_e;
+    float y;
+    gbf16x8 fB[4], hB[4], oB[2], oL[2];
+    uint2 duP[8];
+    auto phase_a = [&]() {
+      asm volatile("" : "+v"(o_w1row), "+v"(o_w2row), "+v"(o_gconst), "+v"(o_b1row));
+      const bf16_t* w1row = reinterpret_cast<const bf16_t*>(gbf_smem + o_w1row);
+      const bf16_t* w2row = reinterpret_cast<const bf16_t*>(gbf_smem + o_w2row);
+      const float* gconst = reinterpret_cast<const float*>(gbf_smem + o_gconst);
+      const float* b1row = reinterpret_cast<const float*>(gbf_smem + o_b1row);
+      if (!valid) {
+#pragma unroll
+        for (int j = 0; j < 16; ++j) gv[j] = 0.f;
+      }
+      oB[0] = gbf_pack8(gv);
+      oB[1] = gbf_pack8(gv + 8);
+      if constexpr (SPLIT_G) {
+        float lo[16];
+#pragma unroll
+        for (int j = 0; j < 16; ++j) lo[j] = gv[j] - (float)oB[j >> 3][j & 7];
+        oL[0] = gbf_pack8(lo);
+        oL[1] = gbf_pack8(lo + 8);
+      }
+      y = sMul[e] * d + sBia[e];
+      if (act) {
+#pragma unroll
+        for (int c = 0; c < 4; ++c) {
+          const float* gc = gconst + 32 * c;
+          fB[c] = gbf_basis8(y, gc, gc + 3 * GBF_K, gc + 2 * GBF_K);
+        }
+#pragma unroll
+        for (int u = 0; u < 4; ++u) {
+          gf32x4 hv[2];
+#pragma unroll
+          for (int hf = 0; hf < 2; ++hf) {
+            const int ft = 2 * u + hf;
+            gf32x4 acc = {0.f, 0.f, 0.f, 0.f}, ua = {0.f, 0.f, 0.f, 0.f};
+#pragma unroll
+            for (int c = 0; c < 2; ++c) {
+              const gbf16x8 wf = *reinterpret_cast<const gbf16x8*>(w2row + 16 * ft * GBF_W2S + 32 * c);
+              acc = __builtin_amdgcn_mfma_f32_16x16x32_bf16(wf, oB[c], acc, 0, 0, 0);
+              if constexpr (SPLIT_G) acc = __builtin_amdgcn_mfma_f32_16x16x32_bf16(wf, oL[c], acc, 0, 0, 0);
+            }
+#pragma unroll
+            for (int c = 0; c < 4; ++c) {
+              const gbf16x8 wf = *reinterpret_cast<const gbf16x8*>(w1row + 16 * ft * GBF_LW + 32 * c);
+              ua = __builtin_amdgcn_mfma_f32_16x16x32_bf16(wf, fB[c], ua, 0, 0, 0);
+            }
+            ua += *reinterpret_cast<const gf32x4*>(b1row + 16 * ft);
+            {
+              f32x2_t y0, g0, y1, g1;
+              gelu_erf_both2(f32x2_t{ua[0], ua[1]}, y0, g0);
+              gelu_erf_both2(f32x2_t{ua[2], ua[3]}, y1, g1);
+              hv[hf] = gf32x4{y0[0], y0[1], y1[0], y1[1]};
+              const uint2 gb = gbf_pack4(gf32x4{g0[0], g0[1], g1[0], g1[1]});
+              acc[0] *= __uint_as_float(gb.x << 16);
+              acc[1] *= __uint_as_float(gb.x & 0xffff0000u);
+              acc[2] *= __uint_as_float(gb.y << 16);
+              acc[3] *= __uint_as_float(gb.y & 0xffff0000u);
+            }
+            duP[ft] = gbf_pack4(acc);
+            __builtin_amdgcn_sched_barrier(0);
+          }
+          float w[8] = {hv[0][0], hv[0][1], hv[0][2], hv[0][3], hv[1][0], hv[1][1], hv[1][2], hv[1][3]};
+          hB[u] = gbf_pack8(w);
+        }
+      } else {
+        const gbf16x8 z = __builtin_bit_cast(gbf16x8, make_uint4(0u, 0u, 0u, 0u));
+#pragma unroll
+        for (int c = 0; c < 4; ++c) fB[c] = hB[c] = z;
+#pragma unroll
+        for (int ft = 0; ft < 8; ++ft) duP[ft] = make_uint2(0u, 0u);
+      }
+    };
+
+    int tile = (int)blockIdx.x * 4 + q4;
+    fetch(tile, act, valid, d, e, gv);
     fetch(tile + stride, n_act, n_valid, n_d, n_e, n_gv);
+    phase_a();
+    auto fold_dy = [&](int pr) {
+      const float dyv = ((sDy[lane] + sDy[GBF_BP + lane]) + sDy[2 * GBF_BP + lane]) + sDy[3 * GBF_BP + lane];
+      const int he = __float_as_int(sEd[pr * GBF_BP + lane]);
+      if (he >= 0) {
+        atomicAdd(&hist[he], dyv * sEd[(2 + pr) * GBF_BP + lane]);
+        atomicAdd(&hist[E + he], dyv);
+      }
+    };
+    bool first = true;
+    int par = 0;
+    for (int base = (int)blockIdx.x * 4; base < ntiles; base += stride, tile += stride) {
+      if (q4 == 0 && !first) fold_dy(par ^ 1);
+      if (g == 0) {
+        sY[ploc] = y;
+        sEd[par * GBF_BP + ploc] = valid ? __int_as_float(e) : __int_as_float(-1);
+        sEd[(2 + par) * GBF_BP + ploc] = d;
+      }
+      first = false;
+      par ^= 1;
+#pragma unroll
+      for (int c = 0; c < 4; ++c) *reinterpret_cast<gbf16x8*>(GBF_SWZ(r0lo, r0hi, 32 * c) + 8 * g) = fB[c];
+#pragma unroll
+      for (int ft = 0; ft < 8; ++ft) *reinterpret_cast<uint2*>(GBF_SWZ(r1lo, r1hi, 16 * ft) + 4 * g) = duP[ft];
+#pragma unroll
+      for (int u = 0; u < 4; ++u) {
+        const uint4 hw = __builtin_bit_cast(uint4, hB[u]);
+        *reinterpret_cast<uint2*>(GBF_SWZ(r2lo, r2hi, 32 * u) + 4 * g) = make_uint2(hw.x, hw.y);
+        *reinterpret_cast<uint2*>(GBF_SWZ(r2lo, r2hi, 32 * u + 16) + 4 * g) = make_uint2(hw.z, hw.w);
+      }
+      *reinterpret_cast<gbf16x8*>(r3lo + 8 * g) = oB[0];
+      *reinterpret_cast<gbf16x8*>(r3lo + 32 + 8 * g) = oB[1];
+      if constexpr (SPLIT_G) {
+        *reinterpret_cast<gbf16x8*>(r3hi + 8 * g) = oL[0];
+        *reinterpret_cast<gbf16x8*>(r3hi + 32 + 8 * g) = oL[1];
+      }
+      __syncthreads();
+      if (base + stride < ntiles) {
+        act = n_act; valid = n_valid; d = n_d; e = n_e;
+#pragma unroll
+        for (int j = 0; j < 16; ++j) gv[j] = n_gv[j];
+        fetch(tile + 2 * stride, n_act, n_valid, n_d, n_e, n_gv);
+        phase_a();
+      }
+      __syncthreads();
+    }
+    if (q4 == 0 && !first) fold_dy(par ^ 1);
+  } else {
+    const int c = q4;
+    const int tswz = (g & 1) << 6;
+    const int trow = (8 * g + (i >> 2)) * GBF_LW + 4 * (i & 3);
+    const bf16_t* const t0lo = T0 + trow + tswz;
+    const bf16_t* const t0hi = T0 + trow + (64 ^ tswz);
+    const bf16_t* const t1w = T0 + TS + trow + ((32 * c) ^ tswz);
+    const bf16_t* const t2w = T0 + 2 * TS + trow + ((32 * c) ^ tswz);
+    const bf16_t* const t3lo = T0 + 3 * TS + trow + tswz;
+    const bf16_t* const t3hi = T0 + 3 * TS + trow + (64 ^ tswz);
+    const int rswz = ((i >> 3) & 1) << 6;
+    const bf16_t* const d1lo = T0 + TS + i * GBF_LW + 8 * g + rswz;
+    const bf16_t* const d1hi = T0 + TS + i * GBF_LW + 8 * g + (64 ^ rswz);
+    unsigned o_w1tr = (unsigned)((8 * g + (i >> 2)) * GBF_LW + 32 * c + 4 * (i & 3)) * 2;
+    unsigned o_kconst = o_f32 + (unsigned)(32 * c + 4 * g) * 4;
     constexpr bool SPLIT_G = sizeof(GT) == 4;
-    gbf16x8 oB[2], oL[2], hB[4];
-    if (!valid) {
-#pragma unroll
-      for (int j = 0; j < 16; ++j) gv[j] = 0.f;
-    }
-    oB[0] = gbf_pack8(gv);
-    oB[1] = gbf_pack8(gv + 8);
-    if constexpr (SPLIT_G) {
-      float lo[16];
-#pragma unroll
-      for (int j = 0; j < 16; ++j) lo[j] = gv[j] - (float)oB[j >> 3][j & 7];
-      oL[0] = gbf_pack8(lo);
-      oL[1] = gbf_pack8(lo + 8);
-    }
-    const float y = sMul[e] * d + sBia[e];
-    if (g == 0) sY[ploc] = y;
-    if (act) {
-      gbf16x8 fB[4];
-#pragma unroll
-      for (int c = 0; c < 4; ++c) {
-        const float* gc = gconst + 32 * c;
-        fB[c] = gbf_basis8(y, gc, gc + 3 * GBF_K, gc + 2 * GBF_K);
-        *reinterpret_cast<gbf16x8*>(GBF_SWZ(r0lo, r0hi, 32 * c) + 8 * g) = fB[c];
-      }
-#pragma unroll
-      for (int u = 0; u < 4; ++u) {
-        gf32x4 hv[2];
-#pragma unroll
-        for (int hf = 0; hf < 2; ++hf) {
-          const int ft = 2 * u + hf;
-          gf32x4 acc = {0.f, 0.f, 0.f, 0.f}, ua = {0.f, 0.f, 0.f, 0.f};
-#pragma unroll
-          for (int c = 0; c < 2; ++c) {
-            const gbf16x8 wf = *reinterpret_cast<const gbf16x8*>(w2row + 16 * ft * GBF_W2S + 32 * c);
-            acc = __builtin_amdgcn_mfma_f32_16x16x32_bf16(wf, oB[c], acc, 0, 0, 0);
-            if constexpr (SPLIT_G) acc = __builtin_amdgcn_mfma_f32_16x16x32_bf16(wf, oL[c], acc, 0, 0, 0);
+    gf32x4 aW1[2][8], aW2[2][4], aB1[2], aB2 = {0.f, 0.f, 0.f, 0.f}, amu[2], asg[2];
+#pragma unroll
+    for (int m = 0; m < 2; ++m) {
+      aB1[m] = amu[m] = asg[m] = gf32x4{0.f, 0.f, 0.f, 0.f};
+#pragma unroll
+      for (int t = 0; t < 8; ++t) aW1[m][t] = gf32x4{0.f, 0.f, 0.f, 0.f};
+#pragma unroll
+      for (int t = 0; t < 4; ++t) aW2[m][t] = gf32x4{0.f, 0.f, 0.f, 0.f};
+    }
+    for (int base = (int)blockIdx.x * 4; base < ntiles; base += stride) {
+      asm volatile("" : "+v"(o_w1tr), "+v"(o_kconst));
+      const bf16_t* w1tr = reinterpret_cast<const bf16_t*>(gbf_smem + o_w1tr);
+      const float* kconst = reinterpret_cast<const float*>(gbf_smem + o_kconst);
+      __syncthreads();
+#define GBF_TFRAG(P, S) gbf_tr8((P) + 32 * (S) * GBF_LW, (P) + (32 * (S) + 4) * GBF_LW)
+#pragma unroll
+      for (int sstep = 0; sstep < 2; ++sstep) {
+        gbf16x8 fa[2];
+#pragma unroll
+        for (int m = 0; m < 2; ++m) {
+          fa[m] = GBF_TFRAG(t1w + 16 * m, sstep);
+          aB1[m] = __builtin_amdgcn_mfma_f32_16x16x32_bf16(fa[m], ones, aB1[m], 0, 0, 0);
+        }
+#pragma unroll
+        for (int kb = 0; kb < 8; ++kb) {
+          const gbf16x8 fb = GBF_TFRAG(GBF_SWZ(t0lo, t0hi, 16 * kb), sstep);
+#pragma unroll
+          for (int m = 0; m < 2; ++m) aW1[m][kb] = __builtin_amdgcn_mfma_f32_16x16x32_bf16(fa[m], fb, aW1[m][kb], 0, 0, 0);
+        }
+      }
+      {
+        gbf16x8 wfr[2][4];
+#pragma unroll
+        for (int m = 0; m < 2; ++m)
+#pragma unroll
+          for (int u = 0; u < 4; ++u) wfr[m][u] = gbf_tr8(w1tr + 16 * m + 32 * u * GBF_LW, w1tr + 16 * m + (32 * u + 4) * GBF_LW);
+#pragma unroll 1
+        for (int j = 0; j < 4; ++j) {
+          gf32x4 acc[2] = {{0.f, 0.f, 0.f, 0.f}, {0.f, 0.f, 0.f, 0.f}};
+#pragma unroll
+          for (int u = 0; u < 4; ++u) {
+            const gbf16x8 dub = *reinterpret_cast<const gbf16x8*>(GBF_SWZ(d1lo, d1hi, 32 * u) + 16 * j * GBF_LW);
+#pragma unroll
+            for (int m = 0; m < 2; ++m) acc[m] = __builtin_amdgcn_mfma_f32_16x16x32_bf16(wfr[m][u], dub, acc[m], 0, 0, 0);
           }
-#pragma unroll
-          for (int c = 0; c < 4; ++c) {
-            const gbf16x8 wf = *reinterpret_cast<const gbf16x8*>(w1row + 16 * ft * GBF_LW + 32 * c);
-            ua = __builtin_amdgcn_mfma_f32_16x16x32_bf16(wf, fB[c], ua, 0, 0, 0);
+          const float yj = sY[16 * j + i];
+          const gf32x2 yy = {yj, yj};
+          gf32x2 dy2 = {0.f, 0.f};
+#pragma unroll
+          for (int m = 0; m < 2; ++m) {
+            const gf32x4 kmu = *reinterpret_cast<const gf32x4*>(kconst + 16 * m);
+            const gf32x4 kis = *reinterpret_cast<const gf32x4*>(kconst + 16 * m + GBF_K);
+            const gf32x4 kcf = *reinterpret_cast<const gf32x4*>(kconst + 16 * m + 2 * GBF_K);
+#define GBF_G2(LO, DV0, DV1)                                                                                   \
+            {                                                                                                  \
+              const gf32x2 is2 = {kis[LO], kis[LO + 1]};                                                       \
+              const gf32x2 z = (yy - gf32x2{kmu[LO], kmu[LO + 1]}) * is2;                                      \
+              const gf32x2 qq = (z * z) * (-0.72134752044448170f);                           \
+              const gf32x2 val = gf32x2{__builtin_amdgcn_exp2f(qq[0]), __builtin_amdgcn_exp2f(qq[1])} * gf32x2{kcf[LO], kcf[LO + 1]}; \
+              const gf32x2 t = gf32x2{DV0, DV1} * val;        \
+              const gf32x2 zs = z * is2;                                                                       \
+              const gf32x2 tz = t * zs;                                                                        \
+              dy2 -= tz;                                                                                       \
+              amu[m][LO] += tz[0]; amu[m][LO + 1] += tz[1];                                                    \
+              const gf32x2 w = t * (z * zs - is2);                                                             \
+              asg[m][LO] += w[0]; asg[m][LO + 1] += w[1];                                                      \
+            }
+            GBF_G2(0, acc[m][0], acc[m][1])
+            GBF_G2(2, acc[m][2], acc[m][3])
+#undef GBF_G2
           }
-          ua += *reinterpret_cast<const gf32x4*>(b1row + 16 * ft);
-          {
-            f32x2_t y0, g0, y1, g1;
-            gelu_erf_both2(f32x2_t{ua[0], ua[1]}, y0, g0);
-            gelu_erf_both2(f32x2_t{ua[2], ua[3]}, y1, g1);
-            hv[hf] = gf32x4{y0[0], y0[1], y1[0], y1[1]};
-            const uint2 gb = gbf_pack4(gf32x4{g0[0], g0[1], g1[0], g1[1]});
-            acc[0] *= __uint_as_float(gb.x << 16);
-            acc[1] *= __uint_as_float(gb.x & 0xffff0000u);
-            acc[2] *= __uint_as_float(gb.y << 16);
-            acc[3] *= __uint_as_float(gb.y & 0xffff0000u);
+          float dy = dy2[0] + dy2[1];
+          dy += __shfl_xor(dy, 16, 64);
+          dy += __shfl_xor(dy, 32, 64);
+          if (g == 0) sDy[c * GBF_BP + 16 * j + i] = dy;
+        }
+      }
+#pragma unroll
+      for (int sstep = 0; sstep < 2; ++sstep) {
+        gbf16x8 fb[2];
+#pragma unroll
+        for (int m = 0; m < 2; ++m) fb[m] = GBF_TFRAG(t2w + 16 * m, sstep);
+#pragma unroll
+        for (int hb = 0; hb < 4; ++hb) {
+          const gbf16x8 fa = GBF_TFRAG(t3lo + 16 * hb, sstep);
+          gbf16x8 fl;
+          if constexpr (SPLIT_G) fl = GBF_TFRAG(t3hi + 16 * hb, sstep);
+#pragma unroll
+          for (int m = 0; m < 2; ++m) {
+            aW2[m][hb] = __builtin_amdgcn_mfma_f32_16x16x32_bf16(fa, fb[m], aW2[m][hb], 0, 0, 0);
+            if constexpr (SPLIT_G) aW2[m][hb] = __builtin_amdgcn_mfma_f32_16x16x32_bf16(fl, fb[m], aW2[m][hb], 0, 0, 0);
           }
-          *reinterpret_cast<uint2*>(GBF_SWZ(r1lo, r1hi, 16 * ft) + 4 * g) = gbf_pack4(acc);
-          __builtin_amdgcn_sched_barrier(0);
-        }
-        float w[8] = {hv[0][0], hv[0][1], hv[0][2], hv[0][3], hv[1][0], hv[1][1], hv[1][2], hv[1][3]};
-        hB[u] = gbf_pack8(w);
-      }
-    } else {
-      const uint4 z4 = make_uint4(0u, 0u, 0u, 0u);
-#pragma unroll
-      for (int c = 0; c < 4; ++c) {
-        *reinterpret_cast<uint4*>(GBF_SWZ(r0lo, r0hi, 32 * c) + 8 * g) = z4;
-        *reinterpret_cast<uint4*>(GBF_SWZ(r1lo, r1hi, 32 * c) + 8 * g) = z4;
-        hB[c] = __builtin_bit_cast(gbf16x8, z4);
-      }
-    }
-    __syncthreads();
-#define GBF_TFRAG(P, S) gbf_tr8((P) + 32 * (S) * GBF_LW, (P) + (32 * (S) + 4) * GBF_LW)
-#pragma unroll
-    for (int sstep = 0; sstep < 4; ++sstep) {
-      const gbf16x8 fa = GBF_TFRAG(t1w, sstep);
-      aB1 = __builtin_amdgcn_mfma_f32_16x16x32_bf16(fa, ones, aB1, 0, 0, 0);
-#pragma unroll
-      for (int kb = 0; kb < 8; ++kb) {
-        const gbf16x8 fb = GBF_TFRAG(GBF_SWZ(t0lo, t0hi, 16 * kb), sstep);
-        aW1[kb] = __builtin_amdgcn_mfma_f32_16x16x32_bf16(fa, fb, aW1[kb], 0, 0, 0);
-      }
-    }
-    {
-      gbf16x8 wfr[4];
-#pragma unroll
-      for (int u = 0; u < 4; ++u) {
-        wfr[u] = gbf_tr8(w1tr + 32 * u * GBF_LW, w1tr + (32 * u + 4) * GBF_LW);
-      }
-      const gf32x4 kmu = *reinterpret_cast<const gf32x4*>(kconst);
-      const gf32x4 kis = *reinterpret_cast<const gf32x4*>(kconst + GBF_K);
-      const gf32x4 kcf = *reinterpret_cast<const gf32x4*>(kconst + 2 * GBF_K);
-#pragma unroll 1
-      for (int j = 0; j < 8; ++j) {
-        gf32x4 acc = {0.f, 0.f, 0.f, 0.f};
-#pragma unroll
-        for (int u = 0; u < 4; ++u) {
-          const gbf16x8 dub = *reinterpret_cast<const gbf16x8*>(GBF_SWZ(d1lo, d1hi, 32 * u) + 16 * j * GBF_LW);
-          acc = __builtin_amdgcn_mfma_f32_16x16x32_bf16(wfr[u], dub, acc, 0, 0, 0);
-        }
-        const float yj = sY[16 * j + i];
-        const gf32x2 yy = {yj, yj};
-        gf32x2 dy2 = {0.f, 0.f};
-#define GBF_G2(LO, DV0, DV1)                                                                                   \
-        {                                                                                                      \
-          const gf32x2 is2 = {kis[LO], kis[LO + 1]};                                                           \
-          const gf32x2 z = (yy - gf32x2{kmu[LO], kmu[LO + 1]}) * is2;                                          \
-          const gf32x2 qq = (z * z) * (-0.72134752044448170f);                               \
-          const gf32x2 val = gf32x2{__builtin_amdgcn_exp2f(qq[0]), __builtin_amdgcn_exp2f(qq[1])} * gf32x2{kcf[LO], kcf[LO + 1]}; \
-          const gf32x2 t = gf32x2{DV0, DV1} * val;          \
-          const gf32x2 zs = z * is2;                                                                           \
-          const gf32x2 tz = t * zs;                                                                            \
-          dy2 -= tz;                                                                                           \
-          amu[LO] += tz[0]; amu[LO + 1] += tz[1];                                                              \
-          const gf32x2 w = t * (z * zs - is2);                                                                 \
-          asg[LO] += w[0]; asg[LO + 1] += w[1];                                                                \
-        }
-        GBF_G2(0, acc[0], acc[1])
-        GBF_G2(2, acc[2], acc[3])
-#undef GBF_G2
-        float dy = dy2[0] + dy2[1];
-        dy += __shfl_xor(dy, 16, 64);
-        dy += __shfl_xor(dy, 32, 64);
-        if (g == 0) atomicAdd(&sDy[16 * j + i], dy);
-      }
-    }
-    __syncthreads();
-#pragma unroll
-    for (int u = 0; u < 4; ++u) {
-      const uint4 hw = __builtin_bit_cast(uint4, hB[u]);
-      *reinterpret_cast<uint2*>(GBF_SWZ(r0lo, r0hi, 32 * u) + 4 * g) = make_uint2(hw.x, hw.y);
-      *reinterpret_cast<uint2*>(GBF_SWZ(r0lo, r0hi, 32 * u + 16) + 4 * g) = make_uint2(hw.z, hw.w);
-    }
-    *reinterpret_cast<gbf16x8*>(r1lo + 8 * g) = oB[0];
-    *reinterpret_cast<gbf16x8*>(r1lo + 32 + 8 * g) = oB[1];
-    if constexpr (SPLIT_G) {
-      *reinterpret_cast<gbf16x8*>(r1hi + 8 * g) = oL[0];
-      *reinterpret_cast<gbf16x8*>(r1hi + 32 + 8 * g) = oL[1];
-    }
-    if (g == 0) {
-      const float dyv = sDy[ploc];
-      sDy[ploc] = 0.f;
-      if (valid) {
-        atomicAdd(&hist[e], dyv * d);
-        atomicAdd(&hist[E + e], dyv);
-      }
-    }
-    __syncthreads();
-#pragma unroll
-    for (int sstep = 0; sstep < 4; ++sstep) {
-      const gbf16x8 fb = GBF_TFRAG(t0w, sstep);
-#pragma unroll
-      for (int hb = 0; hb < 4; ++hb) {
-        const gbf16x8 fa = GBF_TFRAG(t1lo + 16 * hb, sstep);
-        aW2[hb] = __builtin_amdgcn_mfma_f32_16x16x32_bf16(fa, fb, aW2[hb], 0, 0, 0);
+        }
+        const gbf16x8 fo = GBF_TFRAG(t3lo + 16 * c, sstep);
+        aB2 = __builtin_amdgcn_mfma_f32_16x16x32_bf16(fo, ones, aB2, 0, 0, 0);
         if constexpr (SPLIT_G) {
-          const gbf16x8 fl = GBF_TFRAG(t1hi + 16 * hb, sstep);
-          aW2[hb] = __builtin_amdgcn_mfma_f32_16x16x32_bf16(fl, fb, aW2[hb], 0, 0, 0);
-        }
-      }
-      const gbf16x8 fo = GBF_TFRAG(t1lo + 16 * (wave & 3), sstep);
-      aB2 = __builtin_amdgcn_mfma_f32_16x16x32_bf16(fo, ones, aB2, 0, 0, 0);
-      if constexpr (SPLIT_G) {
-        const gbf16x8 fol = GBF_TFRAG(t1hi + 16 * (wave & 3), sstep);
-        aB2 = __builtin_amdgcn_mfma_f32_16x16x32_bf16(fol, ones, aB2, 0, 0, 0);
-      }
-    }
+          const gbf16x8 fol = GBF_TFRAG(t3hi + 16 * c, sstep);
+          aB2 = __builtin_amdgcn_mfma_f32_16x16x32_bf16(fol, ones, aB2, 0, 0, 0);
+        }
+      }
 #undef GBF_TFRAG
+      __syncthreads();
+    }
+    float* const sl = slab ? slab + (long long)blockIdx.x * (GBF_SLAB + 2 * E) : nullptr;
+#pragma unroll
+    for (int m = 0; m < 2; ++m) {
+#pragma unroll
+      for (int kb = 0; kb < 8; ++kb)
+#pragma unroll
+        for (int r = 0; r < 4; ++r) {
+          const int o = (32 * c + 16 * m + 4 * g + r) * GBF_K + 16 * kb + i;
+          if (sl) sl[o] = aW1[m][kb][r]; else atomicAdd(dW1 + o, aW1[m][kb][r]);
+        }
+#pragma unroll
+      for (int hb = 0; hb < 4; ++hb)
+#pragma unroll
+        for (int r = 0; r < 4; ++r) {
+          const int o = (16 * hb + 4 * g + r) * GBF_F + 32 * c + 16 * m + i;
+          if (sl) sl[GBF_F * GBF_K + o] = aW2[m][hb][r]; else atomicAdd(dW2 + o, aW2[m][hb][r]);
+        }
+    }
+    if (i == 0) {
+#pragma unroll
+      for (int r = 0; r < 4; ++r) {
+#pragma unroll
+        for (int m = 0; m < 2; ++m) {
+          const int o = 32 * c + 16 * m + 4 * g + r;
+          if (sl) sl[GBF_SLAB_B1 + o] = aB1[m][r]; else atomicAdd(db1 + o, aB1[m][r]);
+        }
+        const int o = 16 * c + 4 * g + r;
+        if (sl) sl[GBF_SLAB_B2 + o] = aB2[r]; else atomicAdd(db2 + o, aB2[r]);
+      }
+    }
+#pragma unroll
+    for (int m = 0; m < 2; ++m)
+#pragma unroll
+      for (int r = 0; r < 4; ++r) {
+        float a = amu[m][r], sgv = asg[m][r];
+        a += __shfl_xor(a, 1, 64); a += __shfl_xor(a, 2, 64); a += __shfl_xor(a, 4, 64); a += __shfl_xor(a, 8, 64);
+        sgv += __shfl_xor(sgv, 1, 64); sgv += __shfl_xor(sgv, 2, 64); sgv += __shfl_xor(sgv, 4, 64); sgv += __shfl_xor(sgv, 8, 64);
+        if (i == 0) {
+          const int k = 32 * c + 16 * m + 4 * g + r;
+          const float ds = stds[k] < 0.f ? -sgv : sgv;
+          if (sl) { sl[GBF_SLAB_MU + k] = a; sl[GBF_SLAB_SG + k] = ds; }
+          else { atomicAdd(dmeans + k, a); atomicAdd(dstds + k, ds); }
+        }
+      }
+  }
 #undef GBF_SWZ
-    __syncthreads();
-    act = n_act; valid = n_valid; d = n_d; e = n_e;
-#pragma unroll
-    for (int j = 0; j < 16; ++j) gv[j] = n_gv[j];
-  }
+  __syncthreads();
   float* const sl = slab ? slab + (long long)blockIdx.x * (GBF_SLAB + 2 * E) : nullptr;
-#pragma unroll
-  for (int kb = 0; kb < 8; ++kb)
-#pragma unroll
-    for (int r = 0; r < 4; ++r) {
-      const int o = (16 * wave + 4 * g + r) * GBF_K + 16 * kb + i;
-      if (sl) sl[o] = aW1[kb][r]; else atomicAdd(dW1 + o, aW1[kb][r]);
-    }
-#pragma unroll
-  for (int hb = 0; hb < 4; ++hb)
-#pragma unroll
-    for (int r = 0; r < 4; ++r) {
-      const int o = (16 * hb + 4 * g + r) * GBF_F + 16 * wave + i;
-      if (sl) sl[GBF_F * GBF_K + o] = aW2[hb][r]; else atomicAdd(dW2 + o, aW2[hb][r]);
-    }
-  if (i == 0) {
-#pragma unroll
-    for (int r = 0; r < 4; ++r) {
-      const int o = 16 * wave + 4 * g + r;
-      if (sl) {
-        sl[GBF_SLAB_B1 + o] = aB1[r];
-        if (wave < 4) sl[GBF_SLAB_B2 + o] = aB2[r];
-      } else {
-        atomicAdd(db1 + o, aB1[r]);
-        if (wave < 4) atomicAdd(db2 + o, aB2[r]);
-      }
-    }
-  }
-#pragma unroll
-  for (int r = 0; r < 4; ++r) {
-    float a = amu[r], sgv = asg[r];
-    a += __shfl_xor(a, 1, 64); a += __shfl_xor(a, 2, 64); a += __shfl_xor(a, 4, 64); a += __shfl_xor(a, 8, 64);
-    sgv += __shfl_xor(sgv, 1, 64); sgv += __shfl_xor(sgv, 2, 64); sgv += __shfl_xor(sgv, 4, 64); sgv += __shfl_xor(sgv, 8, 64);
-    if (i == 0) {
-      const int k = 16 * wave + 4 * g + r;
-      const float ds = stds[k] < 0.f ? -sgv : sgv;
-      if (sl) { sl[GBF_SLAB_MU + k] = a; sl[GBF_SLAB_SG + k] = ds; }
-      else { atomicAdd(dmeans + k, a); atomicAdd(dstds + k, ds); }
-    }
-  }
-  __syncthreads();
   for (int c = tid; c < E; c += 512) {
     const float a = hist[c], bb = hist[E + c];
     if (sl) { sl[GBF_SLAB + c] = a; sl[GBF_SLAB + E + c] = bb; }
@@ -1189,7 +1245,7 @@
   const int nb = (N + 3) / 4;
   const int tpm = tiled ? nb * nb : cdiv((long long)N * ld, 16);
   const long long ntiles = (long long)B * tpm;
-  const int grid = (int)((ntiles + 7) / 8 < 256 ? (ntiles + 7) / 8 : 256);
+  const int grid = (int)((ntiles + 3) / 4 < 256 ? (ntiles + 3) / 4 : 256);
   const size_t smem = gbf_full_smem(E);
   static bool attr_done = false;
   if (!attr_done) {
diff --git a/scratch/gbf_bwd_bench.py b/scratch/gbf_bwd_bench.py
--- /dev/null
+++ b/scratch/gbf_bwd_bench.py
@@ -0,0 +1,76 @@
+import argparse
+import json
+import os
+import sys
+
+import torch
+
+ROOT = os.path.dirname(os.path.dirname(os.path.abspath(__file__)))
+for p in (ROOT, os.path.join(ROOT, "mm-dti_amd")):
+    if p not in sys.path:
+        sys.path.insert(0, p)
+from mmdti_hip import ops
+
+NAMES = ("dw1", "db1", "dw2", "db2", "dmul", "dbias", "dmeans", "dstds")
+
+
+def inputs(B, N, E=961, K=128, F=128, H=64, seed=7, dev="cuda"):
+    g = torch.Generator(device=dev).manual_seed(seed)
+    dist = torch.rand(B, N, N, generator=g, device=dev) * 8
+    et = torch.randint(0, E, (B, N, N), generator=g, device=dev)
+    mul, bias = 1 + 0.1 * torch.randn(E, generator=g, device=dev), 0.1 * torch.randn(E, generator=g, device=dev)
+    means, stds = torch.rand(K, generator=g, device=dev) * 3, torch.rand(K, generator=g, device=dev) * 3 - 1.5
+    w1 = (torch.randn(F, K, generator=g, device=dev) * 0.2).bfloat16()
+    w2 = (torch.randn(H, F, generator=g, device=dev) * 0.2).bfloat16()
+    b1 = torch.randn(F, generator=g, device=dev) * 0.1
+    gg = ops.pair_tile(torch.randn(B, H, N, N, generator=g, device=dev) * 1e-3, N, 0.0).bfloat16()
+    shapes = ((F, K), (F,), (H, F), (H,), (E,), (E,), (K,), (K,))
+    outs = [torch.zeros(s, device=dev) for s in shapes]
+    return (gg, dist, et, mul, bias, means, stds, w1, b1, w2, ops.pair_ld(N)), outs
+
+
+def main():
+    ap = argparse.ArgumentParser()
+    ap.add_argument("--B", type=int, default=256)
+    ap.add_argument("--N", type=int, default=130)
+    ap.add_argument("--iters", type=int, default=30)
+    ap.add_argument("--warmup", type=int, default=5)
+    ap.add_argument("--save")
+    ap.add_argument("--repeat-check", action="store_true")
+    a = ap.parse_args()
+    args, outs = inputs(a.B, a.N)
+
+    def run():
+        for o in outs:
+            o.zero_()
+        ops.gbf_bias_bwd_full(*args, *[o.view(-1) for o in outs])
+
+    for _ in range(a.warmup):
+        run()
+    torch.cuda.synchronize()
+    first = [o.clone() for o in outs]
+    ts = []
+    for _ in range(a.iters):
+        for o in outs:
+            o.zero_()
+        s, e = torch.cuda.Event(enable_timing=True), torch.cuda.Event(enable_timing=True)
+        s.record()
+        ops.gbf_bias_bwd_full(*args, *[o.view(-1) for o in outs])
+        e.record()
+        e.synchronize()
+        ts.append(s.elapsed_time(e))
+    ts.sort()
+    rec = {"B": a.B, "N": a.N, "lib": os.environ.get("MMDTI_HIP_LIB", "in-tree"), "median_ms": ts[len(ts) // 2], "min_ms": ts[0],
+           "max_ms": ts[-1], "iters": a.iters}
+    if a.repeat_check:
+        rec["repeat_differs"] = [n for n, x, y in zip(NAMES, first, outs) if not torch.equal(x, y)]
+        print(json.dumps(rec))
+        assert not rec["repeat_differs"], "two launches on the same inputs differ"
+    assert all(torch.isfinite(o).all() for o in outs)
+    if a.save:
+        torch.save({n: o.cpu() for n, o in zip(NAMES, outs)}, a.save)
+    print(json.dumps(rec))
+
+
+if __name__ == "__main__":
+    main()
```
